# pinellolab/CRISPResso2

Hardware: NVIDIA H100
Metric: reads/sec aligned+classified (250 bp, single amplicon) (higher is better)
Workload: dtype int32

## Files before the change

### crispresso2_b200/_lib.py

```python
import ctypes as C
import os

import numpy as np

_HERE = os.path.dirname(os.path.abspath(__file__))
DEFAULT_LIB = os.path.join(_HERE, "libc2b200.so")

MAX_Q = 8
MAX_SEEDS = 8
MAX_READ_LEN = 512
MAX_REF_LEN = 1024

F_IGNORE_SUBSTITUTIONS = 1
F_IGNORE_INSERTIONS = 2
F_IGNORE_DELETIONS = 4
F_EXPAND_AMBIGUOUS = 8
F_ASSIGN_FIRST = 16
F_DISCARD_INDEL_READS = 32
F_NO_STRAND_SEARCH = 64
F_NO_PAIRING = 128
F_HDR_REF1 = 256
F_NO_RING = 512
F_LEGACY_INS = 1024
ANN_SAM_OPTIONAL = 1 << 16

ST_BAD_CHAR = 1
ST_UNDEFINED = 2
ST_EDIT_OVERFLOW = 4
E_ARG, E_LIMIT, E_STATE = -2, -3, -4
ST_TOO_LONG = 8

V_ALL_INS, V_ALL_INS_LEFT, V_ALL_DEL, V_ALL_SUB, V_INS, V_DEL, V_SUB, V_SUBBASE0 = range(8)
V_BASEDEV0 = V_SUBBASE0 + MAX_Q
V_INS_LEN = V_BASEDEV0 + MAX_Q + 1
V_DEL_LEN = V_INS_LEN + 1
V_R1_ALL_INS, V_R1_ALL_INS_LEFT, V_R1_ALL_DEL, V_R1_ALL_SUB = V_DEL_LEN + 1, V_DEL_LEN + 2, V_DEL_LEN + 3, V_DEL_LEN + 4
V_R1_BASEDEV0 = V_DEL_LEN + 5
V_INS_NONCODING = V_R1_BASEDEV0 + MAX_Q + 1
V_DEL_NONCODING, V_SUB_NONCODING = V_INS_NONCODING + 1, V_INS_NONCODING + 2
NVEC = V_INS_NONCODING + 3
H_INS_N, H_DEL_N, H_SUB_N, H_EFF_LEN, H_INFRAME, H_FRAMESHIFT, NHIST = range(7)
SCALARS = ["TOTAL", "MODIFIED", "UNMODIFIED", "DISCARDED", "INS", "DEL", "SUB", "ONLY_INS", "ONLY_DEL", "ONLY_SUB",
           "INS_DEL", "INS_SUB", "DEL_SUB", "INS_DEL_SUB", "AMBIGUOUS_W", "N_GLOBAL_SUBS", "N_SUBS_OUTSIDE_WINDOW",
           "N_MODS_IN_WINDOW", "N_MODS_OUTSIDE_WINDOW", "N_READS_IRREGULAR_ENDS", "N_ALIGNED_UNIQUE",
           "N_ALIGNED_COUNT", "REF1_W", "CLASS_MODIFIED", "CLASS_UNMODIFIED", "MOD_FRAMESHIFT", "MOD_NON_FRAMESHIFT",
           "NON_MOD_NON_FRAMESHIFT", "SPLICING_MODIFIED"]
NSCAL = len(SCALARS)
S = {n: k for k, n in enumerate(SCALARS)}


class Params(C.Structure):
    _fields_ = [("gap_open", C.c_int32), ("gap_extend", C.c_int32), ("seed_count", C.c_int32),
                ("seed_min", C.c_int32), ("flags", C.c_uint32), ("nq", C.c_int32),
                ("alphabet", C.c_char * MAX_Q), ("complement", C.c_uint8 * MAX_Q), ("edit_cap", C.c_int32)]


class Ref(C.Structure):
    _fields_ = [("seq", C.c_char_p), ("len", C.c_int32), ("gap_incentive", C.c_void_p),
                ("include_idx", C.c_void_p), ("n_include", C.c_int32), ("min_aln_score", C.c_double),
                ("score_rows", C.c_void_p), ("fw_seeds", C.POINTER(C.c_char_p)), ("rc_seeds", C.POINTER(C.c_char_p)),
                ("n_seeds", C.c_int32), ("tot_exon_len_mod", C.c_int32), ("coding_mask", C.c_void_p)]


ALN_DTYPE = np.dtype([("n_match", "<u2"), ("aln_len", "<u2"), ("score_milli", "<i4"), ("strand", "u1"),
                      ("status", "u1"), ("n_edits", "<u2"), ("insertion_n", "<u2"), ("deletion_n", "<u2"),
                      ("substitution_n", "<u2"), ("n_ins_all", "<u2"), ("n_ins_win", "<u2"), ("n_del_all", "<u2"),
                      ("n_del_win", "<u2"), ("n_del_pos_all", "<u2"), ("n_sub_all", "<u2"),
                      ("irregular_ends", "u1"), ("modified", "u1")])
REC_DTYPE = np.dtype([("winner_mask", "<u4"), ("best_score_milli", "<i4"), ("best_ref", "<i2"), ("n_winners", "u1"),
                      ("ambiguous", "u1"), ("status", "<u4")])
EDIT_DTYPE = np.dtype([("a", "<u2"), ("b", "<u2"), ("type", "u1"), ("in_window", "u1"), ("base", "u1"), ("pad", "u1")])
assert ALN_DTYPE.itemsize == 32 and REC_DTYPE.itemsize == 16 and EDIT_DTYPE.itemsize == 8

EXPORTS = ["c2b_create", "c2b_destroy", "c2b_last_error", "c2b_configure", "c2b_set_edit_cap", "c2b_string_width", "c2b_align_batch",
           "c2b_align_batch_compact", "c2b_ops_words", "c2b_expand_alignment", "c2b_expand_batch", "c2b_ops_device",
           "c2b_align_batch_device", "c2b_set_pair_order", "c2b_sync", "c2b_stream", "c2b_last_kernel_ms", "c2b_launch_count", "c2b_path_counts", "c2b_band_reruns", "c2b_ring_counts", "c2b_diag_counts", "c2b_route_counts",
           "c2b_counts_layout", "c2b_counts_hist_layout", "c2b_counts_reset", "c2b_counts_read", "c2b_counts_device", "c2b_global_align",
           "c2b_classify_aligned", "c2b_classify_aligned_flags", "c2b_host_alloc", "c2b_host_free",
           "c2b_fastq_dedup", "c2b_fastq_dedup_buffer", "c2b_fastq_gpu_available", "c2b_fastq_dedup_gpu", "c2b_fastq_dedup_gpu_buffer", "c2b_sam_dedup_gpu_buffer", "c2b_sam_dedup_buffer", "c2b_fastq_n_reads", "c2b_fastq_n_unique", "c2b_fastq_max_len",
           "c2b_fastq_seqs", "c2b_fastq_offsets", "c2b_fastq_counts", "c2b_fastq_first_index", "c2b_fastq_free",
           "c2b_fastq_last_error", "c2b_fastq_filter", "c2b_fastq_filter_pair", "c2b_rc_merge_weights", "c2b_screen_reads", "c2b_serial_stats",
           "c2b_consensus_from_pairs", "c2b_alleles_build", "c2b_alleles_free", "c2b_alleles_n", "c2b_alleles_order", "c2b_alleles_arena", "c2b_alleles_offsets",
           "c2b_alleles_lengths", "c2b_alleles_write_tsv", "c2b_alleles_around_cut", "c2b_alleles_cut_width", "c2b_alleles_cut_fetch",
           "c2b_annotate_build", "c2b_annotate_free", "c2b_annotate_n", "c2b_annotate_arena", "c2b_annotate_offsets",
           "c2b_annotate_cigar_arena", "c2b_annotate_cigar_offsets", "c2b_annotate_flags", "c2b_annotate_mapq", "c2b_annotate_first",
           "c2b_annotate_last_record", "c2b_annotate_record_arena", "c2b_annotate_record_offsets", "c2b_annotate_write_fastq",
           "c2b_annotate_write_sam", "c2b_annotate_write_sam_passthrough"]

_cache = {}


class LibraryMissing(ImportError):
    pass


def load(path=None):
    path = path or os.environ.get("C2B200_LIB") or DEFAULT_LIB
    if path in _cache:
        return _cache[path]
    if not os.path.exists(path):
        raise LibraryMissing("%s not found: build the CUDA extension first (python -c 'import __graft_entry__ as g; "
                             "g.build()'); crispresso2_b200 has no CPU fallback" % path)
    L = C.CDLL(path)
    vp, i32, i64 = C.c_void_p, C.c_int32, C.c_int64
    L.c2b_create.restype = C.c_int
    L.c2b_create.argtypes = [C.c_int, C.POINTER(vp)]
    L.c2b_destroy.restype = None
    L.c2b_destroy.argtypes = [vp]
    L.c2b_last_error.restype = C.c_char_p
    L.c2b_last_error.argtypes = [vp]
    L.c2b_configure.restype = C.c_int
    L.c2b_configure.argtypes = [vp, C.POINTER(Params), i32, C.POINTER(Ref)]
    L.c2b_set_edit_cap.restype = C.c_int
    L.c2b_set_edit_cap.argtypes = [vp, i32]
    L.c2b_string_width.restype = C.c_int
    L.c2b_string_width.argtypes = [vp, i32]
    L.c2b_align_batch.restype = C.c_int
    L.c2b_align_batch.argtypes = [vp, vp, vp, i64, vp, vp, vp, vp, vp, vp, vp]
    L.c2b_align_batch_compact.restype = C.c_int
    L.c2b_align_batch_compact.argtypes = [vp, vp, vp, i64, vp, vp, vp, vp, vp, vp, vp, vp]
    L.c2b_ops_words.restype = C.c_int
    L.c2b_ops_words.argtypes = [vp, i32]
    L.c2b_expand_alignment.restype = C.c_int
    L.c2b_expand_alignment.argtypes = [vp, vp, C.c_uint32, C.c_char_p, i32, C.c_char_p, i32, vp, vp]
    L.c2b_expand_batch.restype = C.c_int
    L.c2b_expand_batch.argtypes = [vp, vp, vp, i64, vp, vp, vp, i32, vp, i32]
    L.c2b_ops_device.restype = C.c_int
    L.c2b_ops_device.argtypes = [vp, C.POINTER(vp), C.POINTER(vp)]
    L.c2b_align_batch_device.restype = C.c_int
    L.c2b_align_batch_device.argtypes = [vp, vp, vp, i64, i32, vp, vp, vp, vp, vp, vp, vp]
    L.c2b_set_pair_order.restype = C.c_int
    L.c2b_set_pair_order.argtypes = [vp, vp]
    L.c2b_sync.restype = C.c_int
    L.c2b_sync.argtypes = [vp]
    L.c2b_stream.restype = vp
    L.c2b_stream.argtypes = [vp]
    L.c2b_last_kernel_ms.restype = C.c_double
    L.c2b_last_kernel_ms.argtypes = [vp]
    L.c2b_launch_count.restype = i64
    L.c2b_launch_count.argtypes = [vp]
    L.c2b_path_counts.restype = C.c_int
    L.c2b_path_counts.argtypes = [vp, C.POINTER(i64), C.POINTER(i64)]
    L.c2b_band_reruns.restype = i64
    L.c2b_band_reruns.argtypes = [vp]
    L.c2b_ring_counts.restype = C.c_int
    L.c2b_ring_counts.argtypes = [vp, C.POINTER(i64), C.POINTER(i64)]
    L.c2b_diag_counts.restype = C.c_int
    L.c2b_diag_counts.argtypes = [vp, C.POINTER(i64), C.POINTER(i64), C.POINTER(i64)]
    L.c2b_route_counts.restype = C.c_int
    L.c2b_route_counts.argtypes = [vp, C.POINTER(i64), C.POINTER(i64)]
    L.c2b_counts_layout.restype = C.c_int
    L.c2b_counts_layout.argtypes = [vp, C.POINTER(i32), C.POINTER(i32), C.POINTER(i32), C.POINTER(i32)]
    L.c2b_counts_hist_layout.restype = C.c_int
    L.c2b_counts_hist_layout.argtypes = [vp, C.POINTER(i32), C.POINTER(i32), C.POINTER(i32)]
    L.c2b_counts_reset.restype = C.c_int
    L.c2b_counts_reset.argtypes = [vp]
    L.c2b_counts_read.restype = C.c_int
    L.c2b_counts_read.argtypes = [vp, vp, C.c_size_t]
    L.c2b_counts_device.restype = C.c_int
    L.c2b_counts_device.argtypes = [vp, C.POINTER(vp), C.POINTER(C.c_size_t)]
    L.c2b_global_align.restype = C.c_int
    L.c2b_global_align.argtypes = [vp, C.c_char_p, i32, C.c_char_p, i32, C.c_char_p, i32, vp, vp, i32, i32,
                                   C.c_char_p, C.c_char_p, C.POINTER(i32), C.POINTER(i32)]
    L.c2b_classify_aligned.restype = C.c_int
    L.c2b_classify_aligned.argtypes = [vp, C.c_char_p, C.c_char_p, i32, C.c_char_p, i32, vp, i32, vp, vp]
    L.c2b_classify_aligned_flags.restype = C.c_int
    L.c2b_classify_aligned_flags.argtypes = [vp, C.c_char_p, C.c_char_p, i32, C.c_char_p, i32, vp, i32, C.c_uint32, vp, vp]
    L.c2b_host_alloc.restype = vp
    L.c2b_host_alloc.argtypes = [C.c_size_t]
    L.c2b_host_free.restype = None
    L.c2b_host_free.argtypes = [vp]
    L.c2b_fastq_dedup.restype = C.c_int
    L.c2b_fastq_dedup.argtypes = [C.c_char_p, i32, C.POINTER(vp)]
    L.c2b_fastq_dedup_buffer.restype = C.c_int
    L.c2b_fastq_dedup_buffer.argtypes = [vp, C.c_size_t, i32, C.POINTER(vp)]
    for name, rt in (("c2b_fastq_n_reads", i64), ("c2b_fastq_n_unique", i64), ("c2b_fastq_max_len", i32),
                     ("c2b_fastq_seqs", vp), ("c2b_fastq_offsets", vp), ("c2b_fastq_counts", vp),
                     ("c2b_fastq_first_index", vp)):
        getattr(L, name).restype = rt
        getattr(L, name).argtypes = [vp]
    L.c2b_fastq_free.restype = None
    L.c2b_fastq_free.argtypes = [vp]
    L.c2b_consensus_from_pairs.restype = C.c_int
    L.c2b_consensus_from_pairs.argtypes = [C.c_char_p, i32, C.c_char_p, i32, C.c_double, C.c_char_p, i32,
                                           C.c_char_p, i32, C.c_char_p, i32, C.c_double, C.c_char_p, i32,
                                           C.c_char_p, C.c_char_p, C.c_char_p, i32,
                                           C.POINTER(i32), C.POINTER(i32), C.POINTER(i32), C.POINTER(i32)]
    L.c2b_fastq_gpu_available.restype = C.c_int
    L.c2b_fastq_gpu_available.argtypes = []
    L.c2b_fastq_dedup_gpu.restype = C.c_int
    L.c2b_fastq_dedup_gpu.argtypes = [C.c_char_p, i32, C.POINTER(vp)]
    L.c2b_fastq_dedup_gpu_buffer.restype = C.c_int
    L.c2b_fastq_dedup_gpu_buffer.argtypes = [vp, C.c_size_t, i32, C.POINTER(vp)]
    L.c2b_sam_dedup_gpu_buffer.restype = C.c_int
    L.c2b_sam_dedup_gpu_buffer.argtypes = [vp, C.c_size_t, i32, C.POINTER(vp)]
    L.c2b_sam_dedup_buffer.restype = C.c_int
    L.c2b_sam_dedup_buffer.argtypes = [vp, C.c_size_t, i32, C.POINTER(vp)]
    L.c2b_fastq_filter.restype = C.c_int
    L.c2b_fastq_filter.argtypes = [C.c_char_p, C.c_char_p, i32, i32, i32, i32, C.POINTER(i64), C.POINTER(i64)]
    L.c2b_fastq_filter_pair.restype = C.c_int
    L.c2b_fastq_filter_pair.argtypes = [C.c_char_p, C.c_char_p, C.c_char_p, C.c_char_p, i32, i32, i32, i32, C.POINTER(i64), C.POINTER(i64)]
    L.c2b_rc_merge_weights.restype = C.c_int
    L.c2b_rc_merge_weights.argtypes = [vp, vp, i64, vp, vp, vp, i32]
    L.c2b_screen_reads.restype = i64
    L.c2b_screen_reads.argtypes = [vp, vp, i64, i32, vp, i32]
    L.c2b_fastq_last_error.restype = C.c_char_p
    L.c2b_fastq_last_error.argtypes = []
    L.c2b_serial_stats.restype = C.c_int
    L.c2b_serial_stats.argtypes = [vp, vp, vp, i64, i32, vp, vp, i32]
    L.c2b_alleles_build.restype = C.c_int
    L.c2b_alleles_build.argtypes = [vp, vp, vp, vp, i32, i64, vp, vp, vp, vp, i32, C.POINTER(C.c_char_p), vp, vp, i32, C.POINTER(vp)]
    L.c2b_alleles_free.restype = None
    L.c2b_alleles_free.argtypes = [vp]
    L.c2b_alleles_n.restype = i64
    L.c2b_alleles_n.argtypes = [vp]
    for name in ("c2b_alleles_order", "c2b_alleles_arena", "c2b_alleles_offsets", "c2b_alleles_lengths"):
        getattr(L, name).restype = vp
        getattr(L, name).argtypes = [vp]
    L.c2b_alleles_write_tsv.restype = C.c_int
    L.c2b_alleles_write_tsv.argtypes = [vp, C.c_char_p, i64, vp, vp, C.POINTER(C.c_char_p), vp, C.POINTER(C.c_char_p), vp, vp, vp, vp,
                                        C.POINTER(C.c_char_p), i32]
    L.c2b_alleles_around_cut.restype = i64
    L.c2b_alleles_around_cut.argtypes = [vp, i64, vp, i32, i32, i32, vp, vp, vp, vp, vp]
    L.c2b_alleles_cut_width.restype = i32
    L.c2b_alleles_cut_width.argtypes = [vp]
    L.c2b_alleles_cut_fetch.restype = C.c_int
    L.c2b_alleles_cut_fetch.argtypes = [vp, vp, vp, vp, vp, vp, vp, vp, vp, vp]
    cpp = C.POINTER(C.c_char_p)
    L.c2b_annotate_build.restype = C.c_int
    L.c2b_annotate_build.argtypes = [vp, vp, vp, i64, vp, i32, i32, i32, vp, vp, vp, vp, vp, vp, vp, vp, i32, cpp, vp, i32, cpp, cpp, vp,
                                     vp, C.c_uint32, i64, C.POINTER(vp)]
    L.c2b_annotate_free.restype = None
    L.c2b_annotate_free.argtypes = [vp]
    L.c2b_annotate_n.restype = i64
    L.c2b_annotate_n.argtypes = [vp]
    for name in ("c2b_annotate_arena", "c2b_annotate_offsets", "c2b_annotate_cigar_arena", "c2b_annotate_cigar_offsets",
                 "c2b_annotate_flags", "c2b_annotate_mapq", "c2b_annotate_first", "c2b_annotate_last_record",
                 "c2b_annotate_record_arena", "c2b_annotate_record_offsets"):
        getattr(L, name).restype = vp
        getattr(L, name).argtypes = [vp]
    L.c2b_annotate_write_fastq.restype = C.c_int
    L.c2b_annotate_write_fastq.argtypes = [vp, vp, vp, i64, C.c_char_p, C.c_char_p, i32]
    L.c2b_annotate_write_sam.restype = C.c_int
    L.c2b_annotate_write_sam.argtypes = [vp, vp, vp, i64, C.c_char_p, C.c_char_p, C.c_char_p, i32, cpp, cpp, vp, i32]
    L.c2b_annotate_write_sam_passthrough.restype = C.c_int
    L.c2b_annotate_write_sam_passthrough.argtypes = [vp, vp, vp, i64, vp, C.c_size_t, C.c_char_p, i32]
    _cache[path] = L
    return L
```

### crispresso2_b200/csrc/c2b_core.cuh

```cuda
#pragma once
#include <stdint.h>
#include "c2b200.h"

#ifndef C2B_EMU
#include <cuda_runtime.h>
#define C2B_DEV __device__ __forceinline__
#define C2B_DEVNOINL __device__ __noinline__
namespace wp {
C2B_DEV int lane() { return threadIdx.x & 31; }
C2B_DEV int shfl_up(int v, int d) { return __shfl_up_sync(0xffffffffu, v, d); }
C2B_DEV int shfl(int v, int src) { return __shfl_sync(0xffffffffu, v, src); }
C2B_DEV uint32_t shflu(uint32_t v, int src) { return __shfl_sync(0xffffffffu, v, src); }
C2B_DEV uint32_t shflu_up(uint32_t v, int d) { return __shfl_up_sync(0xffffffffu, v, d); }
C2B_DEV int shfl_xor(int v, int m) { return __shfl_xor_sync(0xffffffffu, v, m); }
C2B_DEV uint32_t ballot(bool p) { return __ballot_sync(0xffffffffu, p); }
C2B_DEV void sync() { __syncwarp(); }
#ifdef C2B_X_INLINE_BARRIER
C2B_DEV
#else
__device__ __noinline__
#endif
void grp_sync(int g)
{
    const int w = (int)(threadIdx.x >> 5), sh = 31 - __clz(g);
    const int set = w >> sh;
    asm volatile("barrier.sync %0, %1;" ::"r"(1 + set), "r"(32 << sh) : "memory");
}
C2B_DEV int max3(int a, int b, int c) { return __vimax3_s32(a, b, c); }
C2B_DEV int addmax(int a, int b, int c) { return __viaddmax_s32(a, b, c); }
C2B_DEV uint32_t max3_2(uint32_t a, uint32_t b, uint32_t c) { return __vimax3_s16x2(a, b, c); }
C2B_DEV uint32_t addmax_2(uint32_t a, uint32_t b, uint32_t c) { return __viaddmax_s16x2(a, b, c); }
C2B_DEV uint4 ldg4u(const uint4 *p) { return __ldg(p); }
C2B_DEV void prefetch_l2(const void *p) { asm volatile("prefetch.global.L2 [%0];" ::"l"(p)); }
C2B_DEV int grid_warps() { return (int)(gridDim.x * (blockDim.x >> 5)); }
C2B_DEV uint32_t smem_addr(const void *p) { return (uint32_t)__cvta_generic_to_shared(p); }
C2B_DEV uint32_t lds_u8(uint32_t a) { uint32_t v; asm volatile("ld.shared.u8 %0, [%1];" : "=r"(v) : "r"(a)); return v; }
C2B_DEV uint4 lds_v4(uint32_t a) { uint4 v; asm volatile("ld.shared.v4.u32 {%0,%1,%2,%3}, [%4];" : "=r"(v.x), "=r"(v.y), "=r"(v.z), "=r"(v.w) : "r"(a)); return v; }
C2B_DEV uint2 ldcg2(const uint2 *p) { return __ldcg(p); }
C2B_DEV uint32_t funnel_r(uint32_t lo, uint32_t hi, int sh) { return __funnelshift_r(lo, hi, sh); }
C2B_DEV int popc(uint32_t x) { return __popc(x); }
C2B_DEV int popcll(uint64_t x) { return __popcll(x); }
C2B_DEV int clz(uint32_t x) { return __clz(x); }
C2B_DEV int ffs(uint32_t x) { return __ffs(x); }
C2B_DEV uint32_t ldcg(const uint32_t *p) { return __ldcg(p); }
C2B_DEV int ldcgi(const int *p) { return __ldcg(p); }
C2B_DEV uint64_t ldcg64(const uint64_t *p) { return __ldcg((const unsigned long long *)p); }
C2B_DEV int4 ldg4(const int4 *p) { return __ldg(p); }
C2B_DEV void addg(unsigned long long *p, long long v)
{ asm volatile("red.global.add.u64 [%0], %1;" ::"l"(__cvta_generic_to_global(p)), "l"((unsigned long long)v) : "memory"); }
C2B_DEV void maxg(unsigned long long *p, unsigned long long v)
{ asm volatile("red.global.max.u64 [%0], %1;" ::"l"(__cvta_generic_to_global(p)), "l"(v) : "memory"); }
C2B_DEV uint32_t adds(uint32_t *p, uint32_t v)
{ uint32_t o; asm volatile("atom.shared.add.u32 %0, [%1], %2;" : "=r"(o) : "r"((uint32_t)__cvta_generic_to_shared(p)), "r"(v) : "memory"); return o; }
C2B_DEV unsigned long long fetch_work(unsigned long long *p)
{ unsigned long long o; asm volatile("atom.global.add.u64 %0, [%1], %2;" : "=l"(o) : "l"(__cvta_generic_to_global(p)), "l"(1ull) : "memory"); return o; }
C2B_DEV unsigned long long fetch_add(unsigned long long *p, unsigned long long v)
{ unsigned long long o; asm volatile("atom.global.add.u64 %0, [%1], %2;" : "=l"(o) : "l"(__cvta_generic_to_global(p)), "l"(v) : "memory"); return o; }
}

#else
#include "warp_emu.h"
namespace wp {
C2B_DEV int grid_warps() { return 1; }
}
#endif

namespace c2b {

constexpr int MAXJ = C2B_MAX_READ_LEN;
constexpr int MAXI = C2B_MAX_REF_LEN;
constexpr int OP_M = 0, OP_J = 1, OP_I = 2, OP_NONE = 3;

struct RefDev {
    int32_t I, nrb, kstar, lstar, Ipad;
    int32_t gi0_4;
    int32_t nseeds, seed_len;
    double min_aln;
    const int32_t *prof;
    const int32_t *cIe;
    const int32_t *g4;
    const uint8_t *asc;
    const uint8_t *rcode;
    const uint8_t *incl;
    const uint16_t *cum;
    const uint16_t *cumx, *cums;
    int32_t coding, tem, hist_zero;
    unsigned long long *hist;
    uint64_t fw_seed[C2B_MAX_SEEDS], rc_seed[C2B_MAX_SEEDS];
    unsigned long long *vec;
    unsigned long long *scal;
    int32_t pk_maxJ;
    uint32_t pk_XB, pk_YB, pk_M00;
    const uint32_t *prof2;
    const uint32_t *cIe2;
    const uint32_t *g42;
    int32_t rg_ok, rg_smax, rg_gmax, rg_gsum;
    int32_t dg_ok, dg_S, dg_thr4;
    int32_t dg_c4[2 * 4 + 1];
    int32_t rt_ok, rt_thr;
    int32_t rt_mx;
    int32_t rt_c[32];
    const uint4 *rt_pl;
};
constexpr int32_t RT_OFF = -(1 << 30);
constexpr int RN_DLO = 17, RN_DHI = 11;

struct WorkBlock {
    unsigned long long pair_items, single_items, band_reruns, ring_kept, ring_sent, align_settled;
    unsigned long long diag_proved, diag_listed, tier2, routed, kept;
    struct Launch {
        unsigned long long align_next, tier2_next, general_next;
        unsigned long long widest;
        unsigned long long left_n, tier2_n, narrow_n, diag_n;
    } launch;
};
constexpr size_t WORK_BYTES = 32 * 8;
static_assert(sizeof(WorkBlock) <= WORK_BYTES, "work block");

struct KParams {
    const uint8_t *reads; const int64_t *offsets; int64_t n_reads;
    const int32_t *count, *qweight, *ref_id;
    const int32_t *pair_order;
    c2b_read_rec *recs; c2b_aln_rec *alns; uint8_t *strings; c2b_edit *edits;
    int32_t W, edit_cap;
    const RefDev *refs; int32_t n_refs;
    int32_t out_refs, ops_refs;
    int32_t go, ge, seed_count, seed_min; uint32_t flags; int32_t nq;
    uint8_t alpha[C2B_MAX_Q]; uint8_t comp[C2B_MAX_Q];
    uint32_t *tb; int64_t tb_words_per_warp; int32_t TS;
    uint32_t *tbb; int64_t tbb_words_per_warp;
    uint32_t *tbq;
    int32_t *bnd; int64_t bnd_words_per_warp;
    uint64_t *opsbuf;
    uint64_t *rgops;
    WorkBlock *wb;
    unsigned long long *work_counter;
    uint64_t *gops; uint32_t *gmeta; int32_t NW;
    int32_t *left;
    int32_t *left2;
    int32_t *left0;
    int32_t *left1;
    int32_t route;
    const unsigned long long *n_dev;
    int32_t vstride, hstride;
    const uint32_t *stage_src;
    int32_t stage_bytes;
    const uint8_t *lut;
    int32_t phase_sync;
    const uint64_t *forced_ops;
    const int32_t *forced_n;
};

C2B_DEV int64_t oslot(const KParams &P, int64_t rd, int r) { return rd * P.out_refs + (P.ref_id ? 0 : r); }
C2B_DEV int64_t nreads(const KParams &P) { return P.n_dev ? (int64_t)*P.n_dev : P.n_reads; }

C2B_DEV const RefDev &refdev(const KParams &P, int r) { return P.refs[r]; }

struct WarpSmem {
    uint8_t fw[2][MAXJ];
    uint8_t rc[2][MAXJ];
    uint8_t combo[MAXJ];
    uint8_t rowinfo[MAXI];
    uint32_t rowins[MAXI + 4];
};
constexpr int PK_ROWINFO_STRIDE = 512, PK_ROWINS_STRIDE = 514, PK_MAX_ALN = 512, PK_MAX_ALN2 = 1024;
constexpr int RG_NS = 72, RG_B = 32, RG_MAXD = 8, RG_COMBO = 320;
constexpr int RG_MAX_REFS = 4, RG_OPS_STRIDE = 36;
constexpr int RG_DLO = RG_B + 1, RG_DHI = RG_NS - RG_B - 9;
struct QuadSmem {
    union {
        uint8_t combo[4][RG_COMBO];
        struct { uint64_t ops[4][32]; int32_t n[4][2], err[4][2]; } wk;
    };
};
constexpr int PK_BAND_SLOTS = 64, PK_BAND_B = 28, PK_BAND_MAXD = 8;
struct SlabMode { int slope, off, ns, ring, gb; };

struct Walked { uint64_t ops; int n; int err; uint64_t ops2; };

template <int KSTAR>
C2B_DEV void dp_block(const KParams &P, const RefDev &R, const uint8_t *codes, const int J, const int rb, const int NEG4,
                      uint32_t *__restrict__ tb, const int32_t *bnd_in, int32_t *bnd_out, int &cM, int &cX, int &cY)
{
    const int lane = wp::lane();
    const int nrb = R.nrb, lstar = R.lstar, Ipad = R.Ipad, gi0_4 = R.gi0_4;
    const bool lastblk = (rb == nrb - 1);
    const int nl = lastblk ? lstar + 1 : 32;
    const int rowbase = rb * 256;
    const int r0 = rowbase + 8 * lane;
    const bool islast = lastblk && lane == lstar;
    const int ge4 = 4 * P.ge, d4 = 4 * (P.go - P.ge);

    int M[8], X[8], Y[8], cIe[8], g4[8];
    {
        const int4 *pc = reinterpret_cast<const int4 *>(R.cIe + r0);
        const int4 *pg = reinterpret_cast<const int4 *>(R.g4 + r0);
        int4 a = wp::ldg4(pc), b = wp::ldg4(pc + 1), c = wp::ldg4(pg), d = wp::ldg4(pg + 1);
        cIe[0] = a.x; cIe[1] = a.y; cIe[2] = a.z; cIe[3] = a.w; cIe[4] = b.x; cIe[5] = b.y; cIe[6] = b.z; cIe[7] = b.w;
        g4[0] = c.x; g4[1] = c.y; g4[2] = c.z; g4[3] = c.w; g4[4] = d.x; g4[5] = d.y; g4[6] = d.z; g4[7] = d.w;
    }
#pragma unroll
    for (int k = 0; k < 8; k++) {
        M[k] = NEG4; X[k] = NEG4 | 2; Y[k] = (ge4 * (r0 + k + 1) + gi0_4) | 1;
    }
    int pM, pX, pY;
    if (rb == 0) { pM = 0; pX = NEG4 | 2; pY = NEG4 | 1; }
    else { pM = NEG4; pX = NEG4 | 2; pY = (ge4 * rowbase + gi0_4) | 1; }

    const int nsteps = J + nl - 1;
    const int32_t *__restrict__ prof0 = R.prof + r0;
    uint32_t *__restrict__ tbw = tb + ((int64_t)rb * P.TS) * 32 + lane;
    const bool lane_on = lane < nl;
    int topX = gi0_4 | 2;

    for (int t = 1; t <= nsteps; t++) {
        int uM = wp::shfl_up(M[7], 1), uX = wp::shfl_up(X[7], 1), uY = wp::shfl_up(Y[7], 1);
        const int j = t - lane;
        if (lane == 0) {
            if (rb == 0) { topX += ge4; uM = NEG4; uX = topX; uY = NEG4 | 1; }
            else if (j <= J) { uM = wp::ldcgi(bnd_in + 3 * j); uX = wp::ldcgi(bnd_in + 3 * j + 1); uY = wp::ldcgi(bnd_in + 3 * j + 2); }
        }
        if (lane_on && j >= 1 && j <= J) {
            const int q = codes[j - 1];
            const int4 *pp = reinterpret_cast<const int4 *>(prof0 + q * Ipad);
            const int4 sa = wp::ldg4(pp), sb = wp::ldg4(pp + 1);
            const int s[8] = {sa.x, sa.y, sa.z, sa.w, sb.x, sb.y, sb.z, sb.w};
            const int dcol = (j == J) ? 0 : d4;
            const int dsp = islast ? 0 : dcol;
            int dM = pM, dX = pX, dY = pY;
            int upM = uM, upY = uY;
            uint32_t wT = 0, wIJ = 0;
#pragma unroll
            for (int k = 0; k < 8; k++) {
                const int dik = (k == KSTAR) ? dsp : dcol;
                const int z = wp::max3(dM, dY, dX);
                const int tag = z & 3;
                const int nm = (z - tag) + s[k];
                const int x = wp::addmax(M[k], dik, X[k]) + cIe[k];
                const int y = wp::addmax(upM, dik + g4[k], upY) + ge4;
                wT = wp::funnel_r(wT, (uint32_t)z, 2);
                wIJ = wp::funnel_r(wIJ, (uint32_t)(x | y), 2);
                dM = M[k]; dX = X[k]; dY = Y[k];
                M[k] = nm; X[k] = x | 2; Y[k] = y | 1;
                upM = nm; upY = Y[k];
            }
            tbw[(int64_t)t * 32] = (wT & 0xffff0000u) | (wIJ >> 16);
            if (!lastblk && lane == 31) { bnd_out[3 * j] = M[7]; bnd_out[3 * j + 1] = X[7]; bnd_out[3 * j + 2] = Y[7]; }
        }
        pM = uM; pX = uX; pY = uY;
    }
    if (lastblk) {
        const int k = (KSTAR < 8) ? KSTAR : 0;
        cM = wp::shfl(M[k], lstar); cX = wp::shfl(X[k], lstar); cY = wp::shfl(Y[k], lstar);
    }
}

C2B_DEV void dp_dispatch(const KParams &P, const RefDev &R, const uint8_t *codes, int J, int rb, int NEG4,
                         uint32_t *tb, const int32_t *bi, int32_t *bo, int &cM, int &cX, int &cY)
{
    const int ks = (rb == R.nrb - 1) ? R.kstar : 8;
    switch (ks) {
    case 0: dp_block<0>(P, R, codes, J, rb, NEG4, tb, bi, bo, cM, cX, cY); break;
// ... 1343 lines not shown
```

### crispresso2_b200/csrc/c2b_engine.cu

```cuda
#include <algorithm>
#include <atomic>
#include <mutex>
#ifndef C2B_EMU
#include <sched.h>
#include <sys/syscall.h>
#include <unistd.h>
#include <cctype>
#endif
#include <chrono>
#include <cstdio>
#include <cstdlib>
#include <cstring>
#include <string>
#include <thread>
#include <vector>

#include "c2b_core.cuh"
#include "c2b_split.cuh"
#include "c2b_annotate.cuh"
#include "c2b_fastq_int.h"

using namespace c2b;

#ifndef C2B_EMU
// ... 415 lines not shown
    e->n_refs = n_refs;
    e->refs.assign(n_refs, RefHost());
    e->refdev.assign(n_refs, RefDev());
    int maxI = 0, max_nrb = 1;
    size_t bytes = 0;
    auto al = [](size_t x) { return (x + 255) & ~(size_t)255; };
    std::vector<size_t> base(n_refs);
    for (int r = 0; r < n_refs; r++) {
        const c2b_ref &rf = refs[r];
        if (!rf.seq || rf.len < 1 || !rf.gap_incentive || !rf.score_rows) return fail(e, C2B_E_ARG, "c2b_configure: incomplete reference");
        if (rf.len > C2B_MAX_REF_LEN) return fail(e, C2B_E_LIMIT, "c2b_configure: reference longer than C2B_MAX_REF_LEN");
        if (rf.n_seeds > 0 && (!rf.fw_seeds || !rf.rc_seeds)) return fail(e, C2B_E_ARG, "c2b_configure: seeds missing");
        maxI = std::max(maxI, rf.len);
        const int nrb = (rf.len + 255) / 256, Ipad = nrb * 256;
        max_nrb = std::max(max_nrb, nrb);
        base[r] = bytes;
        bytes += al((size_t)p->nq * Ipad * 4) + 2 * al((size_t)Ipad * 4) + 2 * al(Ipad) + al(Ipad + 1) + 3 * al((size_t)(Ipad + 2) * 2);
        bytes += al((size_t)p->nq * p->nq * Ipad * 4) + 2 * al((size_t)Ipad * 4);
        bytes += al((size_t)(Ipad / 32 + 2) * 16);
    }
    const size_t refs_off = bytes;
    bytes += al(sizeof(RefDev) * n_refs);
    std::vector<unsigned char> blob(bytes, 0);
    if (e->d_tables) { rt_free(e->d_tables); e->d_tables = nullptr; }
    RTCHK(rt_malloc(&e->d_tables, bytes));
    e->vstride = (maxI + 31) & ~31;
    {
        int max_tem = 0;
        for (int r = 0; r < n_refs; r++) max_tem = std::max(max_tem, std::abs((int)refs[r].tot_exon_len_mod));
        if (max_tem > 4 * C2B_MAX_REF_LEN) return fail(e, C2B_E_LIMIT, "c2b_configure: tot_exon_len_mod out of range");
        e->hist_zero = maxI + max_tem;
        const int need = std::max(e->hist_zero + C2B_MAX_READ_LEN + max_tem, std::min(maxI + C2B_MAX_READ_LEN, C2B_MAX_ALN_LEN)) + 1;
        e->hstride = (need + 31) & ~31;
    }
    const size_t per_ref = C2B_NVEC * (size_t)e->vstride + C2B_NHIST * (size_t)e->hstride + C2B_NSCAL;
    e->counts_n = (size_t)n_refs * per_ref;
    if (e->d_counts) { rt_free(e->d_counts); e->d_counts = nullptr; }
    RTCHK(rt_malloc((void **)&e->d_counts, e->counts_n * 8));
    RTCHK(rt_zero(e->d_counts, e->counts_n * 8, e->stream));

    for (int r = 0; r < n_refs; r++) {
        const c2b_ref &rf = refs[r];
        const int I = rf.len, nrb = (I + 255) / 256, Ipad = nrb * 256;
        RefDev &d = e->refdev[r];
        e->refs[r].seq.assign(rf.seq, (size_t)rf.len);
        d.I = I; d.nrb = nrb; d.Ipad = Ipad; d.kstar = (I - 1) & 7; d.lstar = ((I - 1) >> 3) & 31;
        d.min_aln = rf.min_aln_score;
        unsigned char *hb = blob.data() + base[r];
        unsigned char *db = (unsigned char *)e->d_tables + base[r];
        size_t o = 0;
        int32_t *prof = (int32_t *)(hb + o); d.prof = (const int32_t *)(db + o); o += al((size_t)p->nq * Ipad * 4);
        int32_t *cIe = (int32_t *)(hb + o); d.cIe = (const int32_t *)(db + o); o += al((size_t)Ipad * 4);
        int32_t *g4 = (int32_t *)(hb + o); d.g4 = (const int32_t *)(db + o); o += al((size_t)Ipad * 4);
        uint8_t *asc = hb + o; d.asc = db + o; o += al(Ipad);
        uint8_t *rcode = hb + o; d.rcode = db + o; o += al(Ipad);
        uint8_t *incl = hb + o; d.incl = db + o; o += al(Ipad + 1);
        uint16_t *cum = (uint16_t *)(hb + o); d.cum = (const uint16_t *)(db + o); o += al((size_t)(Ipad + 2) * 2);
        uint16_t *cumx = (uint16_t *)(hb + o); d.cumx = (const uint16_t *)(db + o); o += al((size_t)(Ipad + 2) * 2);
        uint16_t *cums = (uint16_t *)(hb + o); d.cums = (const uint16_t *)(db + o); o += al((size_t)(Ipad + 2) * 2);
        uint32_t *prof2 = (uint32_t *)(hb + o); d.prof2 = (const uint32_t *)(db + o); o += al((size_t)p->nq * p->nq * Ipad * 4);
        uint32_t *cIe2 = (uint32_t *)(hb + o); d.cIe2 = (const uint32_t *)(db + o); o += al((size_t)Ipad * 4);
        uint32_t *g42 = (uint32_t *)(hb + o); d.g42 = (const uint32_t *)(db + o); o += al((size_t)Ipad * 4);
        uint4 *rt_pl = (uint4 *)(hb + o); d.rt_pl = (const uint4 *)(db + o); o += al((size_t)(Ipad / 32 + 2) * 16);
        const int64_t lim = (1ll << 27);
        for (int q = 0; q < p->nq; q++)
            for (int i = 0; i < I; i++) {
                const int64_t v = rf.score_rows[(size_t)q * I + i];
                if (v > lim || v < -lim) return fail(e, C2B_E_LIMIT, "c2b_configure: substitution score out of range");
                prof[(size_t)q * Ipad + i] = (int32_t)(4 * v);
            }
        for (int i = 0; i <= I; i++) if (rf.gap_incentive[i] > lim || rf.gap_incentive[i] < -lim) return fail(e, C2B_E_LIMIT, "c2b_configure: gap incentive out of range");
        {
            RefHost &h = e->refs[r];
            h.sabs = h.gabs = h.gsum_abs = 0; h.gi0_abs = std::abs(rf.gap_incentive[0]);
            for (size_t k = 0; k < (size_t)p->nq * I; k++) h.sabs = std::max<int64_t>(h.sabs, std::abs(rf.score_rows[k]));
            for (int i = 0; i <= I; i++) { h.gabs = std::max<int64_t>(h.gabs, std::abs(rf.gap_incentive[i])); h.gsum_abs += std::abs(rf.gap_incentive[i]); }
        }
        for (int row = 0; row < I; row++) {
            cIe[row] = (int32_t)(4 * (p->gap_extend + rf.gap_incentive[row + 1]));
            g4[row] = (int32_t)(4 * rf.gap_incentive[row]);
            asc[row] = (uint8_t)rf.seq[row];
            int code = 255;
            for (int q = 0; q < p->nq; q++) if (rf.seq[row] == p->alphabet[q]) code = q;
            rcode[row] = (uint8_t)code;
        }
        d.gi0_4 = (int32_t)(4 * rf.gap_incentive[0]);
        {
            const int64_t go = p->gap_open, ge = p->gap_extend, beta = -ge, OFFu = 512;
            int64_t gmin = rf.gap_incentive[0], gmax = rf.gap_incentive[0], smin = rf.score_rows[0], smax = rf.score_rows[0];
            for (int i = 0; i <= I; i++) { gmin = std::min(gmin, rf.gap_incentive[i]); gmax = std::max(gmax, rf.gap_incentive[i]); }
            for (size_t k = 0; k < (size_t)p->nq * I; k++) { smin = std::min(smin, rf.score_rows[k]); smax = std::max(smax, rf.score_rows[k]); }
            bool ok = go <= ge && ge <= 0 && gmin >= 0 && gmax <= 64 && smin + 2 * beta >= 0 && smax + 2 * beta <= 1000 &&
                      (go - ge) > -1900 && 4 * (OFFu + (go - ge)) > 256 + 4 * gmax + 3 + 64 && !(p->flags & C2B_F_NO_PAIRING);
            d.pk_maxJ = 0;
            if (ok) {
                for (int J = 1; J <= C2B_MAX_READ_LEN && I + J <= PK_MAX_ALN2; J++) {
                    const int64_t bound = 4 * ((smax + 2 * beta) * std::min(I, J) + gmax * (I + J + 2) + OFFu) + 3;
                    if (bound > 32000) break;
                    d.pk_maxJ = J;
                }
            }
            const uint32_t rep = 0x00010001u;
            d.pk_XB = (uint32_t)((4 * (rf.gap_incentive[0] + OFFu)) | 2) * rep;
            d.pk_YB = (uint32_t)((4 * (rf.gap_incentive[0] + OFFu)) | 1) * rep;
            d.pk_M00 = (uint32_t)(4 * OFFu) * rep;
            {
                int64_t gsum = 0;
                for (int i = 0; i <= I; i++) gsum += rf.gap_incentive[i];
                d.rg_smax = (int32_t)smax; d.rg_gmax = (int32_t)gmax; d.rg_gsum = (int32_t)std::min<int64_t>(gsum, 1 << 24);
                d.rg_ok = d.pk_maxJ > 0 && nrb == 1 && smax >= 0 && 2 * ge + gmax <= smax && gsum < (1 << 24) && !(p->flags & C2B_F_NO_RING);
            }
            if (d.pk_maxJ > 0) {
                for (int qa = 0; qa < p->nq; qa++)
                    for (int qb = 0; qb < p->nq; qb++)
                        for (int i = 0; i < I; i++) {
                            const uint32_t a = (uint32_t)(4 * (rf.score_rows[(size_t)qa * I + i] + 2 * beta));
                            const uint32_t b = (uint32_t)(4 * (rf.score_rows[(size_t)qb * I + i] + 2 * beta));
                            const int rbk = i >> 8, ln = (i >> 3) & 31, hf = (i >> 2) & 1, wd = i & 3;
                            prof2[((size_t)qa * p->nq + qb) * Ipad + rbk * 256 + hf * 128 + ln * 4 + wd] = a | (b << 16);
                        }
                for (int row = 0; row < I; row++) {
                    cIe2[row] = (uint32_t)(4 * rf.gap_incentive[row + 1]) * rep;
                    g42[row] = (uint32_t)(4 * rf.gap_incentive[row]) * rep;
                }
            }
        }
        for (int k = 0; k < rf.n_include; k++) {
            const int64_t v = rf.include_idx[k];
            if (v >= 0 && v < I) incl[v] = 1;
        }
        cum[0] = 0;
        for (int q = 0; q <= Ipad; q++) cum[q + 1] = (uint16_t)(cum[q] + (q < I && incl[q] ? 1 : 0));
        d.coding = rf.coding_mask != nullptr; d.tem = rf.tot_exon_len_mod; d.hist_zero = e->hist_zero;
        {
            const int64_t go = p->gap_open, ge = p->gap_extend, gi0 = rf.gap_incentive[0], gI = rf.gap_incentive[I];
            int64_t gmin = gi0, gp = 0, smax = rf.score_rows[0];
            for (int i = 0; i <= I; i++) { gmin = std::min(gmin, rf.gap_incentive[i]); gp = std::max(gp, rf.gap_incentive[i]); }
            for (size_t k = 0; k < (size_t)p->nq * I; k++) smax = std::max(smax, rf.score_rows[k]);
            int64_t thr = smax * (I - 1) + go + ge + 2 * gp;
            thr = std::max(thr, go * I * I + std::max<int64_t>(smax, 0) * I + 2 * (int64_t)I * gp);
            auto edge_bound = [&](int64_t t) { return smax * (I - t) + t * (2 * ge + gp) + gp; };
            int S = 0;
            while (S < 4 && S + 1 < I && edge_bound(S + 1) > thr) S++;
            if (S + 1 < I) thr = std::max(thr, edge_bound(S + 1));
            thr = std::max<int64_t>(thr, -(1ll << 28));
            d.dg_ok = d.rg_ok && !d.coding && go <= ge && ge <= 0 && gmin >= 0 && 2 * (ge + gp) <= smax && I >= 2 && thr < (1ll << 28) &&
                      !(p->flags & C2B_F_NO_RING);
            d.dg_S = S; d.dg_thr4 = (int32_t)(4 * thr);
            for (int s = -4; s <= 4; s++) {
                const int64_t t = s < 0 ? -s : s;
                d.dg_c4[s + 4] = (int32_t)(4 * (s == 0 ? 0 : 2 * ge * t + gi0 + (s > 0 ? rf.gap_incentive[I - std::min<int64_t>(t, I)] : t * gI)));
            }
            if (!d.dg_ok) { d.dg_S = 0; d.dg_thr4 = 0; }
        }
        {
            const int nq4 = std::min(p->nq, 4);
            for (int i = 0; i < I; i++) {
                const int q = rcode[i];
                if (q >= nq4) continue;
                uint4 &w = rt_pl[i >> 5];
                const uint32_t bit = 1u << (i & 31);
                if (q & 1) w.x |= bit;
                if (q & 2) w.y |= bit;
                w.z |= bit;
            }
            int64_t m = INT64_MAX, x = INT64_MAX;
            for (int q = 0; q < p->nq; q++)
                for (int i = 0; i < I; i++) {
                    const int64_t v = rf.score_rows[(size_t)q * I + i];
                    if (q == rcode[i] && q < nq4) m = std::min(m, v); else x = std::min(x, v);
                }
            const int64_t ge = p->gap_extend, go = p->gap_open, smax = d.rg_smax, gmax = d.rg_gmax, gsum = d.rg_gsum;
            int64_t thr = -(1 << 28);
            if (RN_DHI + 1 <= I) thr = std::max(thr, smax * (I - RN_DHI - 1) + (RN_DHI + 1) * (ge + gmax) + (RN_DHI + 1) * ge + gsum);
            if (RN_DLO + 1 <= I) thr = std::max(thr, smax * (I - RN_DLO - 1) + (RN_DLO + 1) * (ge + gmax) + (RN_DLO + 1) * ge + gsum);
            const int64_t gI = rf.gap_incentive[I];
            const int64_t big = std::max<int64_t>({std::abs(m == INT64_MAX ? 0 : m), std::abs(x == INT64_MAX ? 0 : x), std::abs(go), std::abs(ge), e->refs[r].gabs});
            d.rt_ok = d.dg_ok && I <= 256 && m != INT64_MAX && x != INT64_MAX && m > x && big * (4 * I + 64) < (1ll << 28);
            d.rt_thr = d.rt_ok ? (int32_t)thr : 0;
            d.rt_mx = d.rt_ok ? (int32_t)(m - x) : 0;
            for (int k = 0; k < 32; k++) {
                const int s = k - 16, t = s < 0 ? -s : s;
                const bool on = d.rt_ok && s != 0 && t < I && (s < 0 ? t <= RN_DLO : t <= RN_DHI);
                d.rt_c[k] = RT_OFF;
                if (on) d.rt_c[k] = (int32_t)(go + (t - 1) * ge + (s < 0 ? t * (ge + gI) : t * ge + rf.gap_incentive[I - t]) + x * (I - t));
            }
        }
        if (rf.coding_mask)
            for (int q = 0; q < I; q++) incl[q] |= (uint8_t)((rf.coding_mask[q] & 3) << 1);
        cumx[0] = cums[0] = 0;
        for (int q = 0; q <= Ipad; q++) {
            cumx[q + 1] = (uint16_t)(cumx[q] + (q < I && (incl[q] & 2) ? 1 : 0));
            cums[q + 1] = (uint16_t)(cums[q] + (q < I && (incl[q] & 4) ? 1 : 0));
        }
        const int ns = std::min({(int)rf.n_seeds, (int)p->seed_count, (int)C2B_MAX_SEEDS});
        if (rf.n_seeds > 0 && std::min((int)rf.n_seeds, (int)p->seed_count) > C2B_MAX_SEEDS)
            return fail(e, C2B_E_LIMIT, "c2b_configure: more seeds than C2B_MAX_SEEDS");
        d.nseeds = ns; d.seed_len = 0;
        for (int s = 0; s < C2B_MAX_SEEDS; s++) { d.fw_seed[s] = ~0ull; d.rc_seed[s] = ~0ull; }
        for (int s = 0; s < ns; s++) {
            const std::string f = rf.fw_seeds[s], c = rf.rc_seeds[s];
            if (f.size() != c.size() || f.empty() || f.size() > C2B_MAX_SEED_LEN) return fail(e, C2B_E_LIMIT, "c2b_configure: seed length unsupported");
            if (s && (int)f.size() != d.seed_len) return fail(e, C2B_E_LIMIT, "c2b_configure: seeds of unequal length");
            d.seed_len = (int)f.size();
            d.fw_seed[s] = pack_seed(*p, f); d.rc_seed[s] = pack_seed(*p, c);
        }
        d.vec = e->d_counts + (size_t)r * per_ref;
        d.hist = d.vec + C2B_NVEC * (size_t)e->vstride;
        d.scal = d.hist + C2B_NHIST * (size_t)e->hstride;
    }
    memcpy(blob.data() + refs_off, e->refdev.data(), sizeof(RefDev) * n_refs);
    e->d_refs = (RefDev *)((unsigned char *)e->d_tables + refs_off);
    RTCHK(rt_h2d(e->d_tables, blob.data(), bytes, e->stream));
    RTCHK(rt_sync(e->stream));
    {
        unsigned char lut[256];
        memset(lut, 255, sizeof lut);
        for (int q = 0; q < p->nq; q++) lut[(unsigned char)p->alphabet[q]] = (unsigned char)q;
        int rc2;
        if ((rc2 = ensure(e, e->lut, 256))) return rc2;
        RTCHK(rt_h2d(e->lut.p, lut, 256, e->stream));
        RTCHK(rt_sync(e->stream));
    }
    e->max_I = maxI; e->max_nrb = max_nrb;
    {
        int n_ok = 0;
        for (int r = 0; r < n_refs; r++) n_ok += (e->refdev[r].pk_maxJ > 0 && !e->refdev[r].coding) ? 1 : 0;
        e->split_ok = !(p->flags & (C2B_F_NO_PAIRING | C2B_F_NO_RING)) && n_ok > 0;
        e->split_all = n_ok == n_refs;
        e->diag_any = 0;
        for (int r = 0; r < n_refs; r++) e->diag_any |= e->refdev[r].dg_ok ? 1 : 0;
    }
    e->scratch_TS = 0;
    e->configured = true;
    return C2B_OK;
}

int c2b_set_edit_cap(c2b_engine *e, int32_t edit_cap)
{
    if (!e || !e->configured || edit_cap < 0) return fail(e, C2B_E_ARG, "c2b_set_edit_cap: bad argument");
    e->prm.edit_cap = edit_cap;
    return C2B_OK;
}

int c2b_string_width(const c2b_engine *e, int32_t max_read_len)
{
    if (!e || !e->configured) return C2B_E_STATE;
    return (e->max_I + max_read_len + 31) & ~31;
}

static int ensure_scratch(c2b_engine *e, int maxJ)
{
    const int TS = ((maxJ + 32 + 31) & ~31);
    if (TS <= e->scratch_TS) return C2B_OK;
    int rc;
    auto al = [](size_t x) { return (x + 255) & ~(size_t)255; };
    if ((rc = ensure(e, e->tb, al((size_t)e->n_warps * e->max_nrb * TS * 64 * 4)))) return rc;
    if ((rc = ensure(e, e->tbb, al((size_t)e->n_warps * PK_BAND_SLOTS * 64 * 4)))) return rc;
    if ((rc = ensure(e, e->tbq, al((size_t)e->n_warps * TS * 64 * 4 + 64)))) return rc;
    if ((rc = ensure(e, e->bnd, al((size_t)e->n_warps * 2 * 3 * TS * 4)))) return rc;
    if ((rc = ensure(e, e->ops, al((size_t)e->n_warps * std::min(e->n_refs, (int)C2B_MAX_REFS) * 32 * 8)))) return rc;
    if ((rc = ensure(e, e->rgo, al((size_t)e->n_warps * RG_MAX_REFS * 4 * RG_OPS_STRIDE * 8)))) return rc;
    const bool fresh_work = !e->work.p;
    if ((rc = ensure(e, e->work, WORK_BYTES))) return rc;
    if (fresh_work) RTCHK(rt_zero(e->work.p, WORK_BYTES, e->stream));
    e->scratch_TS = TS;
    return C2B_OK;
}

static int score_range_ok(c2b_engine *e, int64_t maxJ, const char *who)
{
    const int64_t go = std::abs((int64_t)e->prm.gap_open), gap = std::max(go, std::abs((int64_t)e->prm.gap_extend));
    for (int r = 0; r < e->n_refs; r++) {
        const RefHost &h = e->refs[r];
        const int64_t I = (int64_t)h.seq.size(), J = std::max<int64_t>(maxJ, 1);
        const int64_t bound = go * I * J + std::min(I, J) * h.sabs + (I + J) * gap + J * h.gabs + h.gsum_abs + h.gi0_abs;
        if (4 * bound + 3 > (int64_t)INT32_MAX)
            return fail(e, C2B_E_LIMIT, std::string(who) + ": scores, gap penalties and incentives can exceed the int32 range of the DP");
    }
    return C2B_OK;
}

struct Batch {
    const uint8_t *reads; const int64_t *offsets; int64_t n_reads; int32_t max_read_len;
    const int32_t *count, *qweight, *ref_id;
    c2b_read_rec *recs; c2b_aln_rec *alns; uint8_t *strings; c2b_edit *edits;
    uint64_t *gops; uint32_t *gmeta; int32_t *left, *left2, *left0, *left1;
};

struct Switches { bool no_diag, no_route, route_all, no_narrow, no_split; };
static Switches read_switches()
{
    return {getenv("C2B_NO_DIAG") != nullptr, getenv("C2B_NO_ROUTE") != nullptr, getenv("C2B_ROUTE_ALL") != nullptr,
            getenv("C2B_NO_NARROW") != nullptr, getenv("C2B_NO_SPLIT") != nullptr};
}

enum StepKind { STEP_DIAG, STEP_ALIGN, STEP_CLASSIFY, STEP_GENERAL };
struct Step { StepKind kind; KParams P; int grid, block; size_t smem; };
struct Plan { Step step[5]; int n = 0; bool one = false; };

static Plan plan_batch(const c2b_engine *e, const Batch &b, const Switches &sw)
{
    Plan plan;
    WorkBlock *wb = (WorkBlock *)e->work.p;
    KParams P;
    memset(&P, 0, sizeof P);
// ... 92 lines not shown
        wp::g_grp_syncs = 0;
        if (one) emu::run_warp([&]() { process_group<true>(P, S, Q, nullptr, w, 0); });
        else emu::run_warp([&]() { process_group<false>(P, S, Q, nullptr, w, 0); });
        if (P.phase_sync && wp::g_grp_syncs != group_phases(P)) {
            fprintf(stderr, "warp_emu: work group %lld executed %ld phase barriers, expected %d\n", (long long)w, wp::g_grp_syncs, group_phases(P));
            abort();
        }
    }
}

static int run_plan(c2b_engine *, const Plan &plan, rt_stream)
{
    static WarpSmem S; static QuadSmem Q; static ASmem AS; static BSmem BS; static DSmem DS;
    for (int k = 0; k < plan.n; k++) {
        const KParams &P = plan.step[k].P;
        switch (plan.step[k].kind) {
        case STEP_DIAG: emu::run_warp([&]() { diag_loop(P, DS, 0, 1); }); break;
        case STEP_ALIGN: emu::run_warp([&]() { align_loop(P, AS, nullptr, 0); }); break;
        case STEP_CLASSIFY:
            if (plan.one) emu::run_warp([&]() { classify_loop<true>(P, BS, 0, 1); });
            else emu::run_warp([&]() { classify_loop<false>(P, BS, 0, 1); });
            break;
        case STEP_GENERAL:
            if (P.n_dev && plan.one) emu::run_warp([&]() { general_list_loop<true>(P, S, nullptr, 0); });
            else if (P.n_dev) emu::run_warp([&]() { general_list_loop<false>(P, S, nullptr, 0); });
            else run_phase_sets(P, plan.one, S, Q);
            break;
        }
    }
    return C2B_OK;
}
#endif

static int launch_on(c2b_engine *e, rt_stream cs, Batch b)
{
    if (!e || !e->configured) return fail(e, C2B_E_STATE, "c2b_align_batch: engine not configured");
    if (b.n_reads < 0 || !b.recs || !b.alns || (b.n_reads && (!b.reads || !b.offsets))) return fail(e, C2B_E_ARG, "c2b_align_batch: bad argument");
    if (b.n_reads >= (1ll << 31)) return fail(e, C2B_E_LIMIT, "c2b_align_batch: more than 2^31 reads in one batch");
    if (b.max_read_len < 1) b.max_read_len = 1;
    if (b.max_read_len > C2B_MAX_READ_LEN) return fail(e, C2B_E_LIMIT, "c2b_align_batch: read longer than C2B_MAX_READ_LEN");
    if ((int64_t)std::abs((long long)e->prm.gap_open) * b.max_read_len * e->max_I >= (1ll << 28))
        return fail(e, C2B_E_LIMIT, "c2b_align_batch: gap_open * lengths exceeds the int32 score range");
    if (int rc0 = score_range_ok(e, b.max_read_len, "c2b_align_batch")) return rc0;
    if (!b.ref_id && e->n_refs > C2B_MAX_REFS)
        return fail(e, C2B_E_LIMIT, "c2b_align_batch: more than C2B_MAX_REFS references need a per-read ref_id");
    int rc = ensure_scratch(e, b.max_read_len);
    if (rc) return rc;
    if (b.n_reads == 0) return C2B_OK;
    const Plan plan = plan_batch(e, b, read_switches());
    RTCHK(rt_zero(&((WorkBlock *)e->work.p)->launch, sizeof(WorkBlock::Launch), cs));
    if (b.gmeta) RTCHK(rt_zero(b.gmeta, (size_t)b.n_reads * (b.ref_id ? 1 : e->n_refs) * 4, cs));
    if ((rc = run_plan(e, plan, cs))) return rc;
    e->launches += plan.n;
    return C2B_OK;
}

static int ensure_ops(c2b_engine *e, DevBuf &gops, DevBuf &gmeta, DevBuf &left, DevBuf &left2, DevBuf &left0, DevBuf &left1, int64_t n_reads,
                      int nr, int W)
{
    int rc;
    if ((rc = ensure(e, gops, (size_t)n_reads * nr * (W / 32) * 8))) return rc;
    if ((rc = ensure(e, gmeta, (size_t)n_reads * nr * 4))) return rc;
    if ((rc = ensure(e, left, (size_t)(n_reads + 8) * 4))) return rc;
    if ((rc = ensure(e, left2, (size_t)(n_reads + 16) * 4))) return rc;
    if ((rc = ensure(e, left0, (size_t)(n_reads + 16) * 4))) return rc;
    if ((rc = ensure(e, left1, (size_t)(n_reads + 16) * 4))) return rc;
    return C2B_OK;
}

int c2b_align_batch_device(c2b_engine *e, const uint8_t *d_reads, const int64_t *d_offsets, int64_t n_reads,
                           int32_t max_read_len, const int32_t *d_count, const int32_t *d_qweight,
                           const int32_t *d_ref_id, c2b_read_rec *d_recs, c2b_aln_rec *d_alns,
                           uint8_t *d_strings, c2b_edit *d_edits)
{
    if (!e || !e->configured) return fail(e, C2B_E_STATE, "c2b_align_batch_device: engine not configured");
#ifndef C2B_EMU
    cudaSetDevice(e->device);
#endif
    if (max_read_len < 1) max_read_len = 1;
    const int W = (e->max_I + max_read_len + 31) & ~31, nr = d_ref_id ? 1 : e->n_refs;
    int rc = ensure_ops(e, e->gops, e->gmeta, e->left, e->left2, e->left0, e->left1, n_reads, nr, W);
    if (rc) return rc;
    return launch_on(e, e->stream, Batch{d_reads, d_offsets, n_reads, max_read_len, d_count, d_qweight, d_ref_id, d_recs,
                     d_alns, d_strings, d_edits, (uint64_t *)e->gops.p, (uint32_t *)e->gmeta.p, (int32_t *)e->left.p, (int32_t *)e->left2.p,
                     (int32_t *)e->left0.p, (int32_t *)e->left1.p});
}

int c2b_ops_device(c2b_engine *e, void **d_ops, void **d_meta)
{
    if (!e) return C2B_E_ARG;
    if (d_ops) *d_ops = e->gops.p;
    if (d_meta) *d_meta = e->gmeta.p;
    return C2B_OK;
}

int64_t c2b_band_reruns(c2b_engine *e) { return e ? e->band_reruns : 0; }

int c2b_set_pair_order(c2b_engine *e, const int32_t *d_order)
{
    if (!e) return C2B_E_ARG;
    e->pair_order = d_order;
    return C2B_OK;
}

int c2b_sync(c2b_engine *e)
{
    if (!e) return C2B_E_ARG;
    RTCHK(rt_sync(e->stream));
    return C2B_OK;
}

void *c2b_stream(c2b_engine *e) { return e ? (void *)(uintptr_t)e->stream : nullptr; }

double c2b_last_kernel_ms(c2b_engine *e)
{
#ifndef C2B_EMU
    if (!e || !e->launches) return 0.0;
    float ms = 0.f;
    if (cudaEventSynchronize(e->ev1) != cudaSuccess) return 0.0;
    if (cudaEventElapsedTime(&ms, e->ev0, e->ev1) != cudaSuccess) return 0.0;
    return (double)ms;
#else
    (void)e; return 0.0;
#endif
}

int64_t c2b_launch_count(const c2b_engine *e) { return e ? e->launches : 0; }

int c2b_path_counts(c2b_engine *e, int64_t *pair_items, int64_t *single_items)
{
    if (!e || !e->work.p) return fail(e, C2B_E_STATE, "c2b_path_counts: nothing launched yet");
    WorkBlock v;
    RTCHK(rt_d2h(&v, e->work.p, sizeof v, e->stream));
    RTCHK(rt_sync(e->stream));
    e->band_reruns = (int64_t)v.band_reruns; e->ring_pairs = (int64_t)(v.ring_kept + 1) / 2; e->ring_fallbacks = (int64_t)(v.ring_sent + 1) / 2;
    if (getenv("C2B_VERBOSE"))
        fprintf(stderr, "[c2b] counters: general kernel %lld pair items + %lld single items; ALIGN: %lld read x reference combinations kept "
                        "by the ring, %lld sent to the full matrix, %lld reads settled\n", (long long)v.pair_items, (long long)v.single_items,
                (long long)v.ring_kept, (long long)v.ring_sent, (long long)v.align_settled);
    if (pair_items) *pair_items = (int64_t)(v.pair_items + (v.align_settled + 1) / 2);
    if (single_items) *single_items = (int64_t)v.single_items;
    return C2B_OK;
}

int c2b_diag_counts(c2b_engine *e, int64_t *proved, int64_t *tier1, int64_t *tier2)
{
    if (!e || !e->work.p) return fail(e, C2B_E_STATE, "c2b_diag_counts: nothing launched yet");
    WorkBlock v;
    RTCHK(rt_d2h(&v, e->work.p, sizeof v, e->stream));
    RTCHK(rt_sync(e->stream));
    if (proved) *proved = (int64_t)v.diag_proved;
    if (tier1) *tier1 = (int64_t)v.diag_listed;
    if (tier2) *tier2 = (int64_t)v.tier2;
    return C2B_OK;
}

int c2b_route_counts(c2b_engine *e, int64_t *routed, int64_t *kept)
{
    if (!e || !e->work.p) return fail(e, C2B_E_STATE, "c2b_route_counts: nothing launched yet");
    WorkBlock v;
    RTCHK(rt_d2h(&v, e->work.p, sizeof v, e->stream));
    RTCHK(rt_sync(e->stream));
    if (routed) *routed = (int64_t)v.routed;
    if (kept) *kept = (int64_t)v.kept;
    return C2B_OK;
}

int c2b_ring_counts(c2b_engine *e, int64_t *ring_pairs, int64_t *ring_fallbacks)
{
    if (!e) return C2B_E_ARG;
    if (ring_pairs) *ring_pairs = e->ring_pairs;
    if (ring_fallbacks) *ring_fallbacks = e->ring_fallbacks;
    return C2B_OK;
}

static bool is_pageable(const void *p)
{
#ifndef C2B_EMU
    if (!p) return false;
    cudaPointerAttributes a;
    if (cudaPointerGetAttributes(&a, p) != cudaSuccess) { cudaGetLastError(); return true; }
    return a.type == cudaMemoryTypeUnregistered;
#else
    (void)p; return false;
#endif
}

static void par_copy2d(void *dst, size_t dpitch, const void *src, size_t spitch, size_t width, size_t rows)
{
    if (!rows || !width) return;
    const size_t bytes = width * rows;
    int T = bytes > (8u << 20) ? 4 : bytes > (1u << 20) ? 2 : 1;
    auto work = [&](int t) {
        const size_t lo = rows * t / T, hi = rows * (t + 1) / T;
        if (dpitch == width && spitch == width) memcpy((char *)dst + lo * width, (const char *)src + lo * width, (hi - lo) * width);
        else for (size_t r = lo; r < hi; r++) memcpy((char *)dst + r * dpitch, (const char *)src + r * spitch, width);
    };
    std::vector<std::thread> th;
    for (int t = 1; t < T; t++) th.emplace_back(work, t);
    work(0);
    for (auto &x : th) x.join();
}
static void par_copy(void *dst, const void *src, size_t bytes) { par_copy2d(dst, bytes, src, bytes, bytes, 1 == 1 ? (bytes ? 1 : 0) : 0); }

static int ensure_pinned(c2b_engine *e, uint8_t *&p, size_t &cap, size_t n)
{
    if (n <= cap) return C2B_OK;
    if (p) rt_host_free(p);
    const size_t want = n + n / 8 + 4096;
    p = (uint8_t *)rt_host_alloc(want); cap = p ? want : 0;
    return p ? C2B_OK : fail(e, C2B_E_CUDA, "c2b_align_batch: pinned allocation failed");
}

static int align_batch_host(c2b_engine *e, const uint8_t *reads, const int64_t *offsets, int64_t n_reads,
                            const int32_t *count, const int32_t *qweight, const int32_t *ref_id,
                            c2b_read_rec *recs, c2b_aln_rec *alns, uint8_t *strings, uint64_t *ops, uint32_t *meta, c2b_edit *edits)
{
    if (!e || !e->configured) return fail(e, C2B_E_STATE, "c2b_align_batch: engine not configured");
    if (n_reads < 0 || !recs || !alns || (n_reads && (!reads || !offsets))) return fail(e, C2B_E_ARG, "c2b_align_batch: bad argument");
    if ((ops == nullptr) != (meta == nullptr)) return fail(e, C2B_E_ARG, "c2b_align_batch: ops and meta go together");
#ifndef C2B_EMU
    cudaSetDevice(e->device);
#endif
    if (n_reads == 0) return C2B_OK;
    int64_t maxJ = 1, minJ = 0;
    for (int64_t r = 0; r < n_reads; r++) {
        const int64_t L = offsets[r + 1] - offsets[r];
        maxJ = L > maxJ ? L : maxJ;
        minJ = L < minJ ? L : minJ;
    }
    if (minJ < 0) return fail(e, C2B_E_ARG, "c2b_align_batch: offsets not monotone");
    if (maxJ > C2B_MAX_READ_LEN) return fail(e, C2B_E_LIMIT, "c2b_align_batch: read longer than C2B_MAX_READ_LEN");
    if (int rc0 = score_range_ok(e, maxJ, "c2b_align_batch")) return rc0;
    if (!e->pipe_ready) {
        RTCHK(rt_stream_create(&e->s_in));
        RTCHK(rt_stream_create(&e->s_out));
        for (auto &st : e->stage) { RTCHK(rt_event_create(&st.in_done)); RTCHK(rt_event_create(&st.k_done)); RTCHK(rt_event_create(&st.out_done)); }
        e->pipe_ready = true;
    }
    const int W = (e->max_I + (int)maxJ + 31) & ~31, NW = W / 32;
    const int cap = edits ? e->prm.edit_cap : 0;
    const int nr = ref_id ? 1 : e->n_refs;
    const int64_t per_read = (int64_t)nr * (2 * (int64_t)W * (strings ? 1 : 0) + NW * 8 + (int64_t)cap * 8 + 36) + 16 + maxJ + 28;
    int64_t chunk = std::max<int64_t>(4096, std::min<int64_t>((int64_t)(1536ll << 20) / per_read, 1 << 18));
    if (n_reads < 4 * chunk) chunk = std::max<int64_t>(4096, (n_reads + 3) / 4);
    if (const char *v = getenv("C2B_CHUNK")) chunk = std::max<int64_t>(2, atoll(v));
    for (auto &st : e->stage) st.used = false;
    int rc = C2B_OK;
    const bool bounce = getenv("C2B_FORCE_BOUNCE") ? atoi(getenv("C2B_FORCE_BOUNCE")) != 0 : (is_pageable(reads) || is_pageable(recs));
    auto al256 = [](size_t x) { return (x + 255) & ~(size_t)255; };
    struct OutLay { size_t recs, alns, ed, meta, str, ops, total; };
    auto out_layout = [&](int64_t n) {
        OutLay L; size_t o = 0;
        L.recs = o; o = al256(o + (size_t)n * sizeof(c2b_read_rec));
        L.alns = o; o = al256(o + (size_t)n * nr * sizeof(c2b_aln_rec));
        L.ed = o; o = al256(o + (size_t)n * nr * cap * sizeof(c2b_edit));
        L.meta = o; o = al256(o + (meta ? (size_t)n * nr * 4 : 0));
        L.str = o; o = al256(o + (strings ? (size_t)n * nr * 2 * W : 0));
        L.ops = o; o = al256(o + (ops ? (size_t)n * nr * NW * 8 : 0));
        L.total = o;
        return L;
    };
    struct Pending { bool any = false; int64_t c0 = 0, n = 0; int set = 0; } pend;
    auto flush = [&](const Pending &q) -> int {
        c2b_engine::Stage &st = e->stage[q.set];
        const OutLay L = out_layout(q.n);
        int rc2;
        if (bounce && (rc2 = ensure_pinned(e, st.h_out, st.h_out_cap, L.total))) return rc2;
        uint8_t *ho = st.h_out;
        RTCHK(rt_wait(e->s_out, st.k_done));
        RTCHK(rt_d2h(bounce ? (void *)(ho + L.recs) : (void *)(recs + q.c0), st.recs.p, (size_t)q.n * sizeof(c2b_read_rec), e->s_out));
        RTCHK(rt_d2h(bounce ? (void *)(ho + L.alns) : (void *)(alns + q.c0 * nr), st.alns.p, (size_t)q.n * nr * sizeof(c2b_aln_rec), e->s_out));
        if (cap) RTCHK(rt_d2h(bounce ? (void *)(ho + L.ed) : (void *)(edits + q.c0 * nr * cap), st.ed.p, (size_t)q.n * nr * cap * sizeof(c2b_edit), e->s_out));
        if (meta) RTCHK(rt_d2h(bounce ? (void *)(ho + L.meta) : (void *)(meta + q.c0 * nr), st.gmeta.p, (size_t)q.n * nr * 4, e->s_out));
        size_t Wt = 0;
        if (strings || ops) {
            RTCHK(rt_event_sync(st.k_done));
            long long wmax = 0;
            RTCHK(rt_d2h(&wmax, (const char *)st.maxlen.p, 8, e->s_out));
            RTCHK(rt_sync(e->s_out));
            Wt = ((size_t)wmax + 31) & ~(size_t)31;
            if (Wt > (size_t)W) Wt = W;
            if (strings) RTCHK(rt_d2h_2d((bounce ? ho + L.str : strings + q.c0 * nr * 2 * W) + (W - Wt), (const uint8_t *)st.str.p + (W - Wt), W, Wt, (size_t)q.n * nr * 2, e->s_out));
            if (ops) RTCHK(rt_d2h_2d(bounce ? (void *)(ho + L.ops) : (void *)(ops + q.c0 * nr * NW), st.gops.p, (size_t)NW * 8, Wt / 32 * 8, (size_t)q.n * nr, e->s_out));
        }
        RTCHK(rt_record(st.out_done, e->s_out));
        st.drain = bounce; st.d_c0 = q.c0; st.d_n = q.n; st.d_Wt = Wt;
        return C2B_OK;
    };
    auto drain = [&](c2b_engine::Stage &st) -> int {
        if (!st.drain) return C2B_OK;
        RTCHK(rt_event_sync(st.out_done));
        const int64_t c0 = st.d_c0, n = st.d_n;
        const OutLay L = out_layout(n);
        const uint8_t *ho = st.h_out;
        par_copy(recs + c0, ho + L.recs, (size_t)n * sizeof(c2b_read_rec));
        par_copy(alns + c0 * nr, ho + L.alns, (size_t)n * nr * sizeof(c2b_aln_rec));
        if (cap) par_copy(edits + c0 * nr * cap, ho + L.ed, (size_t)n * nr * cap * sizeof(c2b_edit));
        if (meta) par_copy(meta + c0 * nr, ho + L.meta, (size_t)n * nr * 4);
        if (strings) par_copy2d(strings + c0 * nr * 2 * W + (W - st.d_Wt), W, ho + L.str + (W - st.d_Wt), W, st.d_Wt, (size_t)n * nr * 2);
        if (ops) par_copy2d(ops + c0 * nr * NW, (size_t)NW * 8, ho + L.ops, (size_t)NW * 8, st.d_Wt / 32 * 8, (size_t)n * nr);
        st.drain = false;
        return C2B_OK;
    };
    std::vector<int64_t> cuts;
    {
// ... 480 lines not shown
```

### crispresso2_b200/csrc/c2b_split.cuh

```cuda
#pragma once
#include "c2b_core.cuh"

namespace c2b {

constexpr uint32_t GM_NONE = 0, GM_ALIGNED = 1;

C2B_DEV uint32_t gmeta_pack(int n, int strand, uint32_t state) { return (uint32_t)n | ((uint32_t)strand << 16) | (state << 24); }

struct ASmem {
    uint8_t fw[2][RG_COMBO], rc[2][RG_COMBO];
    uint8_t combo[8][RG_COMBO];
    uint32_t fin[96];
    uint8_t lut[256];
};

C2B_DEV void asmem_init(const KParams &P, ASmem &S)
{
    const int lane = wp::lane();
    for (int k = lane; k < 256; k += 32) S.lut[k] = P.lut[k];
    wp::sync();
}

C2B_DEV int64_t read_at(const KParams &P, int64_t idx) { return P.pair_order ? (int64_t)P.pair_order[idx] : idx; }

C2B_DEV void leftover_pair(const KParams &P, int64_t rdA, int64_t rdB)
{
    if (wp::lane() == 0) {
        const unsigned long long pos = wp::fetch_add(&P.wb->launch.left_n, 2ull);
        P.left[pos] = (int32_t)rdA; P.left[pos + 1] = (int32_t)rdB;
    }
}

C2B_DEV void leftover_one(const KParams &P, int64_t rd)
{
    if (wp::lane() == 0) { const unsigned long long pos = wp::fetch_add(&P.wb->launch.left_n, 1ull); P.left[pos] = (int32_t)rd; }
}

C2B_DEV bool load_codes_a(const KParams &P, const uint8_t *lut, int64_t off, int J, uint8_t *fw, uint8_t *rc)
{
    const int lane = wp::lane();
    bool bad = false;
    for (int base = 0; base < J; base += 128) {
        uint8_t ch[4];
#pragma unroll
        for (int e = 0; e < 4; e++) { const int p = base + lane + 32 * e; ch[e] = p < J ? P.reads[off + p] : (uint8_t)P.alpha[0]; }
#pragma unroll
        for (int e = 0; e < 4; e++) {
            const int p = base + lane + 32 * e;
            int code = lut[ch[e]];
            if (code == 255) { bad = true; code = 0; }
            if (p < J) { fw[p] = (uint8_t)code; rc[J - 1 - p] = P.comp[code]; }
        }
    }
    return wp::ballot(bad) != 0;
}

template <int RL = 8, int NP = 4>
C2B_DEV void walk_ring4(const KParams &P, const RefDev &R, const int *Jq, const uint2 *__restrict__ tb2, const int *s0, uint32_t mask,
                        Walked *out, const int q0 = 0)
{
    constexpr int NS = 9 * RL, B = 4 * RL;
    const int lane = wp::lane();
    const int hl = lane & 15, hb = lane & 16;
    const int TS = P.TS;
    int i[NP], j[NP], s[NP], n[NP], err[NP];
    uint32_t acc[NP], lo[NP], hi[NP];
#pragma unroll
    for (int q = 0; q < NP; q++) {
        const bool on = (mask >> q) & 1u;
        i[q] = on ? R.I : 0; j[q] = on ? Jq[q] : 0; s[q] = s0[q]; n[q] = 0; err[q] = 0; acc[q] = 0; lo[q] = hi[q] = ~0u;
    }
#define C2B_PUSH4(q, op_, cnt_) do { int cnt = (cnt_); const uint32_t pat = (uint32_t)(op_) * 0x55555555u;                          \
        while (cnt > 0) { const int room = 16 - (n[q] & 15); const int c = cnt < room ? cnt : room;                                  \
            acc[q] = (uint32_t)((((uint64_t)pat << 32) | acc[q]) >> (2 * c)); n[q] += c; cnt -= c;                                   \
            if ((n[q] & 15) == 0) { const int ix = (n[q] >> 4) - 1; if (hl == (ix >> 1)) { if (ix & 1) hi[q] = acc[q]; else lo[q] = acc[q]; } } } } while (0)
    for (;;) {
        uint2 w2[NP]; bool valid[NP], inband[NP]; int sh[NP];
        bool anyact = false;
#pragma unroll
        for (int q = 0; q < NP; q++) {
            const bool active = i[q] > 0 && j[q] > 0;
            anyact |= active;
            const int di = (s[q] != OP_I), dj = (s[q] != OP_J);
            const int ci = i[q] - hl * di, cj = j[q] - hl * dj;
            valid[q] = active && ci >= 1 && cj >= 1;
            inband[q] = valid[q];
            w2[q] = make_uint2(0u, 0u); sh[q] = 0;
            if (valid[q]) {
                const int r = ci - 1, l = (r >> 3) & 31;
                const int slot = cj + l - 9 * l + B;
                inband[q] = (unsigned)slot < (unsigned)NS;
                sh[q] = 2 * (7 - (r & 7));
                if (inband[q]) w2[q] = wp::ldcg2(tb2 + (int64_t)(RL * (q0 + q) + (l & (RL - 1))) * TS + cj + l);
            }
        }
        if (!wp::ballot(anyact)) break;
#pragma unroll
        for (int q = 0; q < NP; q++) {
            const bool active = i[q] > 0 && j[q] > 0;
            const uint32_t w = hb ? ((w2[q].x & 0xffff0000u) | (w2[q].y >> 16)) : ((w2[q].x << 16) | (w2[q].y & 0xffffu));
            const uint32_t v = (valid[q] && inband[q]) ? (w >> sh[q]) : 0u;
            const int tag = (int)((v >> 16) & 3u);
            const bool cont = valid[q] && (s[q] == OP_M ? tag == OP_M : (v & (uint32_t)s[q]) != 0u);
            const uint32_t bc = (wp::ballot(cont) >> hb) & 0xffffu, bv = (wp::ballot(valid[q]) >> hb) & 0xffffu;
            const uint32_t bo = (wp::ballot(valid[q] && !inband[q]) >> hb) & 0xffffu;
            int nvalid = wp::popc(bv);
            if (bo) { const int fo = wp::ffs(bo) - 1; if (fo < nvalid) nvalid = fo; }
            const bool miss = active && nvalid == 0;
            int f = wp::ffs(~bc) - 1;
            if (f < 0 || f > nvalid) f = nvalid;
            const bool brk = f < nvalid;
            const int run = brk ? f + 1 : nvalid;
            const int tagf = wp::shfl(tag, hb + (f < 16 ? f : 15));
            if (miss) { err[q] |= 4; i[q] = 0; j[q] = 0; }
            else if (active) {
                const int di = (s[q] != OP_I), dj = (s[q] != OP_J);
                const int news = brk ? (s[q] == OP_M ? tagf : OP_M) : s[q];
                C2B_PUSH4(q, s[q], run);
                i[q] -= run * di; j[q] -= run * dj;
                err[q] |= (news == 3);
                s[q] = news;
            }
        }
    }
#pragma unroll
    for (int q = 0; q < NP; q++) {
        if (j[q] > 0 && s[q] != OP_I) err[q] |= 1;
        if (i[q] > 0 && s[q] != OP_J) err[q] |= 1;
        while (j[q] > 0) { const int c = j[q] < 32 ? j[q] : 32; C2B_PUSH4(q, OP_I, c); j[q] -= c; }
        while (i[q] > 0) { const int c = i[q] < 32 ? i[q] : 32; C2B_PUSH4(q, OP_J, c); i[q] -= c; }
        if (n[q] & 15) {
            const int ix = n[q] >> 4, used = 2 * (n[q] & 15);
            const uint32_t a = (acc[q] >> (32 - used)) | (~0u << used);
            if (hl == (ix >> 1)) { if (ix & 1) hi[q] = a; else lo[q] = a; }
        }
        out[q].ops = (uint64_t)lo[q] | ((uint64_t)hi[q] << 32); out[q].ops2 = ~0ull; out[q].n = n[q]; out[q].err = err[q];
    }
#undef C2B_PUSH4
}

C2B_DEV int match_count_half(const KParams &P, const RefDev &R, const uint8_t *codes, int J, const Walked &wk)
{
    const int hl = wp::lane() & 15;
    const uint64_t lo = 0x5555555555555555ull;
    int base_i = R.I, base_j = J, match = 0;
#pragma unroll 1
    for (int word = 0; word < 2; word++) {
        const uint64_t ops = word ? wk.ops2 : wk.ops;
        const int ci = 32 - wp::popcll((ops >> 1) & lo);
        const int cj = 32 - wp::popcll(ops & lo);
        int pk = (ci << 16) | cj;
#pragma unroll
        for (int d = 1; d < 16; d <<= 1) { const int v = wp::shfl_up(pk, d); if (hl >= d) pk += v; }
        const int tot = wp::shfl(pk, (wp::lane() & 16) | 15);
        pk -= (ci << 16) | cj;
        int i = base_i - (pk >> 16), j = base_j - (pk & 0xffff);
        uint64_t rest = ops;
#pragma unroll 4
        for (int e = 0; e < 32; e++) {
            const int op = (int)rest & 3;
            rest >>= 2;
            if (op == OP_NONE) continue;
            if (op == OP_M && (uint32_t)P.alpha[codes[j - 1]] == (uint32_t)R.asc[i - 1]) match++;
            i -= (op != OP_I); j -= (op != OP_J);
        }
        base_i -= tot >> 16; base_j -= tot & 0xffff;
    }
#pragma unroll
    for (int d = 8; d >= 1; d >>= 1) match += wp::shfl_xor(match, d);
    return match;
}

C2B_DEV void align_group(const KParams &P, ASmem &S, const uint32_t *staged_prof, int64_t wq, int warp_slot)
{
    const int lane = wp::lane(), g = lane >> 3;
    const int64_t first = 4 * wq;
    const bool multi = P.ref_id == nullptr && P.n_refs > 1;
    bool quad = (P.tbq != nullptr || P.tb != nullptr) && 2 * first + 7 < nreads(P) && (!multi || P.n_refs <= RG_MAX_REFS);
    int r0 = 0;
    uint32_t ringmask = 0;
    if (quad) {
        const int x = lane & 7;
        const int64_t rd = read_at(P, 2 * first + x);
        const int Jx = (int)(P.offsets[rd + 1] - P.offsets[rd]);
        const int rx = P.ref_id ? P.ref_id[rd] : 0;
        r0 = wp::shfl(rx, 0);
        const int Jn = wp::shfl_xor(Jx, 1);
        bool ok = rx == r0 && Jx == Jn && Jx >= 1 && Jx <= RG_COMBO && Jx + 32 <= P.TS;
        const int k0 = multi ? 0 : r0, k1 = multi ? P.n_refs : r0 + 1;
        for (int k = k0; k < k1; k++) {
            const RefDev &R = refdev(P, k);
            ok = ok && !R.coding && Jx <= R.pk_maxJ;
            const bool rk = P.tbq != nullptr && R.rg_ok && R.I + Jx <= PK_MAX_ALN && Jx - R.I <= RG_MAXD && R.I - Jx <= RG_MAXD;
            if (wp::ballot(rk) == 0xffffffffu) ringmask |= 1u << (k - k0);
        }
        quad = wp::ballot(ok) == 0xffffffffu;
        if (!P.tb && ringmask != (k1 - k0 >= 32 ? 0xffffffffu : (1u << (k1 - k0)) - 1u)) quad = false;
    }
    if (!quad) {
#pragma unroll 1
        for (int q = 0; q < 4; q++) {
            if (2 * (first + q) >= nreads(P)) break;
            const int64_t rdA = read_at(P, 2 * (first + q));
            if (2 * (first + q) + 1 < nreads(P)) leftover_pair(P, rdA, read_at(P, 2 * (first + q) + 1));
            else leftover_one(P, rdA);
        }
        return;
    }
    const int k0 = multi ? 0 : r0, k1 = multi ? P.n_refs : r0 + 1;
    uint2 *tbq = P.tbq ? reinterpret_cast<uint2 *>(P.tbq + (int64_t)warp_slot * P.TS * 64) : nullptr;
    uint32_t okmask = 0, modes = 0;
    uint32_t both2[RG_MAX_REFS] = {0, 0, 0, 0};
    int Jg = 0, Jmax = 0;
#pragma unroll 1
    for (int q = 0; q < 4; q++) {
        const int64_t rdA = read_at(P, 2 * (first + q)), rdB = read_at(P, 2 * (first + q) + 1);
        const int J = (int)(P.offsets[rdA + 1] - P.offsets[rdA]);
        bool bad = false;
#pragma unroll 1
        for (int x = 0; x < 2; x++) bad |= load_codes_a(P, S.lut, P.offsets[x ? rdB : rdA], J, S.fw[x], S.rc[x]);
        wp::sync();
        int mAB = 0; bool agree = true;
        uint32_t bothq[RG_MAX_REFS] = {0, 0, 0, 0};
#pragma unroll 1
        for (int k = k0; k < k1; k++) {
            int m = 0;
#pragma unroll 1
            for (int x = 0; x < 2; x++) m |= strand_mode(P, refdev(P, k), S.fw[x], J) << (2 * x);
            if (k == k0) mAB = m;
#pragma unroll
            for (int x = 0; x < 2; x++) {
                const int mk = (m >> (2 * x)) & 3, m0 = (mAB >> (2 * x)) & 3;
                if (mk == 2) bothq[(k - k0) & (RG_MAX_REFS - 1)] |= 1u << x;
                else if (mk != (m0 == 2 ? 0 : m0)) agree = false;
            }
        }
        const int mA = mAB & 3, mB = mAB >> 2;
        if (!bad && agree) {
            const uint8_t *cA = mA == 1 ? S.rc[0] : S.fw[0], *cB = mB == 1 ? S.rc[1] : S.fw[1];
            for (int p = lane; p < J; p += 32) S.combo[q][p] = (uint8_t)(cA[p] * P.nq + cB[p]);
            okmask |= 1u << q; modes |= (uint32_t)mAB << (4 * q);
#pragma unroll
            for (int kk = 0; kk < RG_MAX_REFS; kk++) both2[kk] |= bothq[kk] << (2 * q);
            if (g == q) Jg = J;
            if (J > Jmax) Jmax = J;
        }
        wp::sync();
    }
    uint32_t good2 = 0;
#pragma unroll
    for (int q = 0; q < 4; q++) if ((okmask >> q) & 1u) good2 |= 3u << (2 * q);
    if (!P.tb) {
#pragma unroll
        for (int kk = 0; kk < RG_MAX_REFS; kk++) { good2 &= ~both2[kk]; both2[kk] = 0; }
    }
    int npass = 0, ntried = 0, nboth = 0;
#pragma unroll 1
    for (int k = k0; k < k1 && good2; k++) {
        const RefDev &R = refdev(P, k);
        const uint32_t bothk = both2[(k - k0) & (RG_MAX_REFS - 1)];
        const uint32_t ring2 = good2 & ~bothk;
        nboth += wp::popc(bothk & good2);
        const bool staged = (k == 0 && staged_prof != nullptr);
        uint32_t pass2 = 0;
        if (((ringmask >> (k - k0)) & 1u) && ring2) {
        if (staged) dp_ring<true>(P, R, staged_prof, S.combo[g], Jg, Jmax + R.lstar, tbq, S.fin);
        else dp_ring<false>(P, R, R.prof2, S.combo[g], Jg, Jmax + R.lstar, tbq, S.fin);
        wp::sync();
        const int fl = 3 * ((lane & 24) | (R.lstar & 7));
        const uint32_t cM = Jg > 0 ? S.fin[fl] : PK_SENT, cX = Jg > 0 ? S.fin[fl + 1] : PK_SENT, cY = Jg > 0 ? S.fin[fl + 2] : PK_SENT;
        wp::sync();
        const uint32_t z = wp::max3_2(cM, cY, cX);
        const uint32_t s2 = z & PK_TM;
        const int thr = ring_bound(P, R, Jg) + 512 - P.ge * (R.I + Jg);
        const bool passA = Jg > 0 && (int)((z & 0xffffu) >> 2) > thr, passB = Jg > 0 && (int)(z >> 18) > thr;
        const uint32_t bA = wp::ballot(passA), bB = wp::ballot(passB);
#pragma unroll
        for (int q = 0; q < 4; q++) pass2 |= (((bA >> (8 * q)) & 1u) | (((bB >> (8 * q)) & 1u) << 1)) << (2 * q);
        pass2 &= ring2;
        ntried += wp::popc(ring2);
        {
            int Jq[4], s0[4];
            Walked wk4[4];
            uint32_t walkmask = 0;
#pragma unroll
            for (int q = 0; q < 4; q++) {
                const uint32_t sq = wp::shflu(s2, 8 * q);
                Jq[q] = wp::shfl(Jg, 8 * q);
                s0[q] = (lane & 16) ? (int)(sq >> 16) : (int)(sq & 3u);
                if ((pass2 >> (2 * q)) & 3u) walkmask |= 1u << q;
            }
            walk_ring4(P, R, Jq, tbq, s0, walkmask, wk4);
#pragma unroll
            for (int q = 0; q < 4; q++) {
                if (!((walkmask >> q) & 1u)) continue;
                const Walked &wk = wk4[q];
                const uint32_t eb = wp::ballot(wk.err != 0);
                if (eb & 0xffffu) pass2 &= ~(1u << (2 * q));
                if (eb >> 16) pass2 &= ~(2u << (2 * q));
                const int h = lane >> 4, hl = lane & 15;
                if (!((pass2 >> (2 * q + h)) & 1u)) continue;
                const int64_t rd = read_at(P, 2 * (first + q) + h);
                const int64_t slot = oslot(P, rd, k);
                if (hl < P.NW) P.gops[slot * P.NW + hl] = wk.ops;
                if (hl == 0) {
                    const int mode = (int)((modes >> (4 * q + 2 * h)) & 3u);
                    P.gmeta[slot] = gmeta_pack(wk.n, mode == 1, GM_NONE);
                }
            }
        }
        npass += wp::popc(pass2);
        } else ntried += wp::popc(ring2);
        const uint32_t failed = ring2 & ~pass2;
        if ((failed | (bothk & good2)) && P.tb) {
            uint2 *tb2 = reinterpret_cast<uint2 *>(P.tb + (int64_t)warp_slot * P.tb_words_per_warp);
            int32_t *bnd = P.bnd + (int64_t)warp_slot * P.bnd_words_per_warp;
            const int h = lane >> 4, hl = lane & 15;
#pragma unroll 1
            for (int job = 0; job < 16; job++) {
                const int q = job >> 2, kind = job & 3;
                if (kind == 3) continue;
                const uint32_t fq = (failed >> (2 * q)) & 3u;
                const uint32_t bq = ((bothk & good2) >> (2 * q)) & 3u;
                if (kind == 0 ? fq == 0 : !((bq >> (kind - 1)) & 1u)) continue;
                const int Jp = wp::shfl(Jg, 8 * q);
                const uint8_t *combo = S.combo[q];
                wp::sync();
                if (kind) {
                    const int64_t rdx = read_at(P, 2 * (first + q) + (kind - 1));
                    load_codes_a(P, S.lut, P.offsets[rdx], Jp, S.fw[0], S.rc[0]);
                    wp::sync();
                    for (int p = lane; p < Jp; p += 32) S.fw[1][p] = (uint8_t)(S.fw[0][p] * P.nq + S.rc[0][p]);
                    combo = S.fw[1];
                    wp::sync();
                }
                const Walked wk = align_pair(P, R, staged ? staged_prof : R.prof2, staged, combo, Jp, tb2, nullptr, bnd);
                const uint32_t eb = wp::ballot(wk.err != 0);
                if (kind == 0) {
                    const bool mine = ((fq >> h) & 1u) && !((h ? (eb >> 16) : (eb & 0xffffu)));
                    if (mine) {
                        const int64_t rd = read_at(P, 2 * (first + q) + h);
                        const int64_t slot = oslot(P, rd, k);
                        if (hl < P.NW) P.gops[slot * P.NW + hl] = wk.ops;
                        if (hl + 16 < P.NW) P.gops[slot * P.NW + 16 + hl] = wk.ops2;
                        if (hl == 0) P.gmeta[slot] = gmeta_pack(wk.n, (int)((modes >> (4 * q + 2 * h)) & 3u) == 1, GM_NONE);
                    }
                    const uint32_t mb = wp::ballot(mine);
                    if (mb & 0xffffu) pass2 |= 1u << (2 * q);
                    if (mb >> 16) pass2 |= 2u << (2 * q);
                } else {
                    const int nm = match_count_half(P, R, h ? S.rc[0] : S.fw[0], Jp, wk);
                    const int sc = score_milli(nm, wk.n > 0 ? wk.n : 1);
                    const int sc_fw = wp::shfl(sc, 0), sc_rc = wp::shfl(sc, 16);
                    const int pick = sc_rc > sc_fw ? 1 : 0;
                    const uint32_t bit = 1u << (2 * q + kind - 1);
                    if (eb) good2 &= ~bit;
                    else if (h == pick) {
                        const int64_t rd = read_at(P, 2 * (first + q) + (kind - 1));
                        const int64_t slot = oslot(P, rd, k);
                        if (hl < P.NW) P.gops[slot * P.NW + hl] = wk.ops;
                        if (hl + 16 < P.NW) P.gops[slot * P.NW + 16 + hl] = wk.ops2;
                        if (hl == 0) P.gmeta[slot] = gmeta_pack(wk.n, pick, GM_NONE);
                    }
                }
            }
        }
        pass2 |= bothk & good2;
        good2 &= pass2;
        wp::sync();
    }
#ifndef C2B_EMU
    if (tbq && ringmask) {
        const char *base = reinterpret_cast<const char *>(tbq);
        const int64_t bytes = (int64_t)P.TS * 64 * 4;
        for (int64_t o = (int64_t)lane * 128; o < bytes; o += 32 * 128)
            asm volatile("discard.global.L2 [%0], 128;" ::"l"(base + o) : "memory");
    }
#endif
    if (lane == 0) {
        wp::addg(&P.wb->align_settled, wp::popc(good2));
        wp::addg(&P.wb->ring_kept, npass);
        wp::addg(&P.wb->ring_sent, ntried - npass + nboth + 2 * (k1 - k0) * (4 - wp::popc(okmask)));
    }
#pragma unroll 1
    for (int q = 0; q < 4; q++) {
        const int64_t rdA = read_at(P, 2 * (first + q)), rdB = read_at(P, 2 * (first + q) + 1);
        const uint32_t gq = (good2 >> (2 * q)) & 3u;
        if (gq) {
            const int64_t rd = (lane & 1) ? rdB : rdA;
            const int k = k0 + (lane >> 1);
            if (k < k1 && ((gq >> (lane & 1)) & 1u)) { const int64_t slot = oslot(P, rd, k); P.gmeta[slot] = (P.gmeta[slot] & 0x00ffffffu) | (GM_ALIGNED << 24); }
        }
        if (gq == 0) leftover_pair(P, rdA, rdB);
        else if (gq != 3u) leftover_one(P, gq == 1u ? rdB : rdA);
    }
}

C2B_DEV bool align_narrow16(const KParams &P, ASmem &S, const uint32_t *staged_prof, int64_t w16, int warp_slot)
{
    constexpr int RL = 4, DLO = 4 * RL + 1, DHI = 9 * RL - 4 * RL - 9;
    static_assert(DLO == RN_DLO && DHI == RN_DHI, "the diagonal tier's routing test assumes this band");
    const int lane = wp::lane(), g = lane >> 2;
    const int64_t first = 16 * w16;
    if (!P.left2 || P.tbq == nullptr || first + 15 >= nreads(P) || (P.ref_id == nullptr && P.n_refs > 1)) return false;
    int r0, J0;
    {
        const int64_t rd = read_at(P, first + (lane & 15));
        const int Jx = (int)(P.offsets[rd + 1] - P.offsets[rd]);
        const int rx = P.ref_id ? P.ref_id[rd] : 0;
        r0 = wp::shfl(rx, 0); J0 = wp::shfl(Jx, 0);
        const RefDev &R = refdev(P, r0);
        const bool ok = rx == r0 && Jx == J0 && Jx >= 1 && Jx <= RG_COMBO && Jx + 32 <= P.TS && R.rg_ok && !R.coding && Jx <= R.pk_maxJ &&
                        R.I + Jx <= PK_MAX_ALN && Jx - R.I <= RG_MAXD && R.I - Jx <= RG_MAXD;
        if (wp::ballot(ok) != 0xffffffffu) return false;
    }
    const RefDev &R = refdev(P, r0);
    const int J = J0;
    uint2 *tbq = reinterpret_cast<uint2 *>(P.tbq + (int64_t)warp_slot * P.TS * 64);
    uint32_t modes = 0, use2 = 0;
#pragma unroll 1
    for (int q = 0; q < 8; q++) {
        const int64_t rdA = read_at(P, first + 2 * q), rdB = read_at(P, first + 2 * q + 1);
        bool badA = load_codes_a(P, S.lut, P.offsets[rdA], J, S.fw[0], S.rc[0]);
        bool badB = load_codes_a(P, S.lut, P.offsets[rdB], J, S.fw[1], S.rc[1]);
        wp::sync();
        int m = 0;
#pragma unroll 1
        for (int x = 0; x < 2; x++) m |= strand_mode(P, R, S.fw[x], J) << (2 * x);
        const int mA = m & 3, mB = m >> 2;
        const uint8_t *cA = mA == 1 ? S.rc[0] : S.fw[0], *cB = mB == 1 ? S.rc[1] : S.fw[1];
        for (int p = lane; p < J; p += 32) S.combo[q][p] = (uint8_t)(cA[p] * P.nq + cB[p]);
        modes |= (uint32_t)m << (4 * q);
        if (!badA && mA != 2) use2 |= 1u << (2 * q);
        if (!badB && mB != 2) use2 |= 2u << (2 * q);
        wp::sync();
    }
    const bool staged = (r0 == 0 && staged_prof != nullptr);
    if (staged) dp_ring<true, RL>(P, R, staged_prof, S.combo[g], J, J + R.lstar, tbq, S.fin);
    else dp_ring<false, RL>(P, R, R.prof2, S.combo[g], J, J + R.lstar, tbq, S.fin);
    wp::sync();
    const int fl = 3 * ((lane & ~(RL - 1)) | (R.lstar & (RL - 1)));
    const uint32_t cM = S.fin[fl], cX = S.fin[fl + 1], cY = S.fin[fl + 2];
    wp::sync();
    const uint32_t z = wp::max3_2(cM, cY, cX);
    const uint32_t s2 = z & PK_TM;
    const int thr = ring_bound(P, R, J, DLO, DHI) + 512 - P.ge * (R.I + J);
    const uint32_t bA = wp::ballot((int)((z & 0xffffu) >> 2) > thr), bB = wp::ballot((int)(z >> 18) > thr);
    uint32_t pass2 = 0;
#pragma unroll
    for (int q = 0; q < 8; q++) pass2 |= (((bA >> (RL * q)) & 1u) | (((bB >> (RL * q)) & 1u) << 1)) << (2 * q);
    pass2 &= use2;
#pragma unroll 1
    for (int half = 0; half < 2; half++) {
        const int q0 = 4 * half;
        int Jq[4], s0[4];
        Walked wk4[4];
        uint32_t walkmask = 0;
#pragma unroll
        for (int q = 0; q < 4; q++) {
            const uint32_t sq = wp::shflu(s2, RL * (q0 + q));
            Jq[q] = J;
            s0[q] = (lane & 16) ? (int)(sq >> 16) : (int)(sq & 3u);
            if ((pass2 >> (2 * (q0 + q))) & 3u) walkmask |= 1u << q;
        }
        if (!walkmask) continue;
        walk_ring4<RL, 4>(P, R, Jq, tbq, s0, walkmask, wk4, q0);
#pragma unroll
        for (int q = 0; q < 4; q++) {
            if (!((walkmask >> q) & 1u)) continue;
            const int qq = q0 + q;
            const Walked &wk = wk4[q];
            const uint32_t eb = wp::ballot(wk.err != 0);
            if (eb & 0xffffu) pass2 &= ~(1u << (2 * qq));
            if (eb >> 16) pass2 &= ~(2u << (2 * qq));
            const int h = lane >> 4, hl = lane & 15;
            if (!((pass2 >> (2 * qq + h)) & 1u)) continue;
            const int64_t rd = read_at(P, first + 2 * qq + h);
            const int64_t slot = oslot(P, rd, r0);
            if (hl < P.NW) P.gops[slot * P.NW + hl] = wk.ops;
            if (hl == 0) P.gmeta[slot] = gmeta_pack(wk.n, (int)((modes >> (4 * qq + 2 * h)) & 3u) == 1, GM_ALIGNED);
        }
    }
#ifndef C2B_EMU
    {
        const char *base = reinterpret_cast<const char *>(tbq);
        const int64_t bytes = (int64_t)P.TS * 64 * 4;
        for (int64_t o = (int64_t)lane * 128; o < bytes; o += 32 * 128)
            asm volatile("discard.global.L2 [%0], 128;" ::"l"(base + o) : "memory");
    }
#endif
    const uint32_t rest = 0xffffu & ~pass2;
    if (lane < 16 && ((rest >> lane) & 1u)) {
        const unsigned long long pos = wp::fetch_add(&P.wb->launch.tier2_n, 1ull);
        P.left2[pos] = (int32_t)read_at(P, first + lane);
    }
    if (lane == 0) {
        wp::addg(&P.wb->align_settled, wp::popc(pass2));
        wp::addg(&P.wb->ring_kept, wp::popc(pass2));
        wp::addg(&P.wb->tier2, 16 - wp::popc(pass2));
    }
    return true;
}

C2B_DEV void align_loop(const KParams &P, ASmem &S, const uint32_t *staged_prof, int warp)
{
    const int lane = wp::lane();
    asmem_init(P, S);
    const int64_t nrd = nreads(P);
    const unsigned ahead = (unsigned)wp::grid_warps();
    if (P.left2) {
        const unsigned total = (unsigned)((nrd + 15) / 16);
        for (;;) {
            unsigned w = 0;
            if (lane == 0) w = (unsigned)wp::fetch_work(P.work_counter);
            w = (unsigned)wp::shfl((int)w, 0);
            if (w >= total) break;
            if (w + ahead < total) {
                const int64_t g = (int64_t)w + ahead;
                if (!P.pair_order) {
                    const int64_t last = 16 * g + 16 < nrd ? 16 * g + 16 : nrd;
                    const int64_t a = P.offsets[16 * g] + (int64_t)lane * 128;
                    if (a < P.offsets[last]) wp::prefetch_l2(P.reads + a);
                } else {
                    const int64_t x = 16 * g + (lane >> 1);
                    if (x < nrd) {
                        const int64_t rd = read_at(P, x);
                        const int64_t b1 = P.offsets[rd + 1];
                        for (int64_t a = (P.offsets[rd] & ~(int64_t)127) + (int64_t)(lane & 1) * 128; a < b1; a += 256)
                            wp::prefetch_l2(P.reads + a);
                    }
                }
            }
            if (!align_narrow16(P, S, staged_prof, (int64_t)w, warp)) {
                align_group(P, S, staged_prof, 2 * (int64_t)w, warp);
                wp::sync();
                if (8 * (2 * (int64_t)w + 1) < nrd) align_group(P, S, staged_prof, 2 * (int64_t)w + 1, warp);
            }
            wp::sync();
        }
        return;
    }
    const unsigned total = (unsigned)((nrd + 7) / 8);
    for (;;) {
        unsigned w = 0;
        if (lane == 0) w = (unsigned)wp::fetch_work(P.work_counter);
        w = (unsigned)wp::shfl((int)w, 0);
        if (w >= total) break;
        if (w + ahead < total && !P.pair_order) {
            const int64_t g = (int64_t)w + ahead;
            const int64_t last = 8 * g + 8 < nrd ? 8 * g + 8 : nrd;
            const int64_t a = P.offsets[8 * g] + (int64_t)lane * 128;
            if (a < P.offsets[last]) wp::prefetch_l2(P.reads + a);
        }
        align_group(P, S, staged_prof, (int64_t)w, warp);
        wp::sync();
    }
}

constexpr int B_RD_BYTES = 32 * 16;

static_assert(C2B_NSCAL <= 32, "one lane per scalar slot");
template <int NA> struct ScAcc { long long v[NA]; int ref[NA]; unsigned wmax; };

template <int NA>
C2B_DEV void sc_init(ScAcc<NA> &A)
{
#pragma unroll
    for (int x = 0; x < NA; x++) { A.v[x] = 0; A.ref[x] = -1; }
    A.wmax = 0;
}

template <int NA>
C2B_DEV void sc_acc(ScAcc<NA> &A, const KParams &P, int r, int slot, long long val)
{
    const int lane = wp::lane();
    const int k = NA == 1 ? 0 : (r & (NA - 1));
#pragma unroll
// ... 361 lines not shown
    rec.best_ref = (int16_t)r;
    RowOut o; o.ins_n = o.del_n = o.sub_n = 0; o.n_ins_all = o.n_ins_win = o.n_del_all = o.n_del_win = 0;
    o.n_del_pos = o.n_sub_all = 0; o.nent = 0;
    c2b_edit *ed = P.edits ? P.edits + oslot(P, rd, r) * (int64_t)P.edit_cap : nullptr;
    const bool counted = !ambiguous && (!first || nth == 0) && w > 0;
    const bool len_inline = counted && !two_scans && !ign_i && !ign_d;
    scan(o, ed, RM_SCAL | ((counted && !two_scans) ? RM_VEC : 0) | (len_inline ? RM_LEN : 0));
    const bool has_d = !ign_d && o.del_n > 0, has_i = !ign_i && o.ins_n > 0, has_s = !ign_s && o.sub_n > 0;
    const bool modified = has_d || has_i || has_s;
    uint32_t astatus = 0;
    if (P.edits && o.nent > P.edit_cap) astatus |= C2B_ST_EDIT_OVERFLOW;
    if (counted) {
        const bool discard = two_scans && (o.del_n > 0 || o.ins_n > 0);
        if (discard) sc_acc(A, P, r, C2B_S_DISCARDED, w);
        else {
            const bool entered = modified || R.tem != 0;
            const bool lenv = !len_inline && entered && (o.n_ins_win > 0 || o.n_del_win > 0);
            if (two_scans || lenv) scan(o, nullptr, (two_scans ? RM_VEC : 0) | (lenv ? RM_LEN : 0));
            if (entered) edited_update_acc(A, P, R, r, o, w);
            sc_acc(A, P, r, C2B_S_TOTAL, w);
            sc_acc(A, P, r, modified ? C2B_S_MODIFIED : C2B_S_UNMODIFIED, w);
        }
    } else if (ambiguous && nth == 0 && w > 0) sc_acc(A, P, r, C2B_S_AMBIGUOUS_W, w);
    if (counted && (two_scans || expand)) {
        const bool discarded = two_scans && (o.del_n > 0 || o.ins_n > 0), joined = !ONE && expand && !first && rec.n_winners > 1;
        if (discarded != joined) sc_acc(A, P, r, modified ? C2B_S_CLASS_MODIFIED : C2B_S_CLASS_UNMODIFIED, discarded ? w : -w);
    }
    int irr = 0;
    if (lane == 0) {
        c2b_aln_rec b = multi ? load_aln(P.alns + oslot(P, rd, r)) : a;
        b.insertion_n = (uint16_t)o.ins_n; b.deletion_n = (uint16_t)o.del_n; b.substitution_n = (uint16_t)o.sub_n;
        b.n_ins_all = (uint16_t)o.n_ins_all; b.n_ins_win = (uint16_t)o.n_ins_win;
        b.n_del_all = (uint16_t)o.n_del_all; b.n_del_win = (uint16_t)o.n_del_win;
        b.n_del_pos_all = (uint16_t)o.n_del_pos; b.n_sub_all = (uint16_t)o.n_sub_all;
        b.n_edits = (uint16_t)o.nent; b.modified = modified; b.status |= (uint8_t)astatus;
        irr = b.irregular_ends;
        P.alns[oslot(P, rd, r)] = b;
    }
    irr = wp::shfl(irr, 0);
    rec.status |= astatus;
    const bool is_last = (rec.winner_mask >> (r & 31)) >> 1 == 0;
    if (is_last) {
        const long long total_mods = o.n_ins_all + o.n_del_pos + o.n_sub_all;
        const long long in_win = o.sub_n + o.del_n + o.ins_n;
        sc_acc(A, P, r, C2B_S_N_GLOBAL_SUBS, cnt * o.n_sub_all);
        sc_acc(A, P, r, C2B_S_N_SUBS_OUTSIDE_WINDOW, cnt * (o.n_sub_all - o.sub_n));
        sc_acc(A, P, r, C2B_S_N_MODS_IN_WINDOW, cnt * in_win);
        sc_acc(A, P, r, C2B_S_N_MODS_OUTSIDE_WINDOW, cnt * (total_mods - in_win));
        if (irr) sc_acc(A, P, r, C2B_S_N_READS_IRREGULAR_ENDS, cnt);
        sc_acc(A, P, r, C2B_S_N_ALIGNED_UNIQUE, 1);
        sc_acc(A, P, r, C2B_S_N_ALIGNED_COUNT, cnt);
    }
}

template <bool ONE>
C2B_DEV void classify_read(const KParams &P, int64_t rd, const BPre &pre, const BSmem &S, ScAcc<ONE ? 1 : RG_MAX_REFS> &A)
{
    const int lane = wp::lane();
    const int r_begin = pre.r_begin;
    const int r_end = r_begin + pre.nref;
    const int64_t off = pre.off;
    const int J = pre.J;
    const bool multi = !ONE && (r_end - r_begin) > 1;

    c2b_read_rec rec; rec.winner_mask = 0; rec.best_score_milli = -1000; rec.best_ref = -1; rec.n_winners = 0;
    rec.ambiguous = 0; rec.status = 0;
    ColCtx cx[ONE ? 1 : RG_MAX_REFS];
    c2b_aln_rec a; init_aln(a, 0);
#pragma unroll 1
    for (int r = r_begin; r < r_end; r++) {
        const RefDev &R = refdev(P, r);
        const int64_t slot = oslot(P, rd, r);
        ColCtx &c = cx[ONE ? 0 : r - r_begin];
        const uint32_t gm = pre.gm[ONE ? 0 : r - r_begin];
        c.ops = S.ops[ONE ? 0 : r - r_begin]; c.rd = S.rd + (int)((uintptr_t)(P.reads + off) & 15); c.n = (int)(gm & 0xffffu); c.J = J; c.strand = (int)((gm >> 16) & 1u);
        uint8_t *o_read = P.strings ? P.strings + (slot * 2) * (int64_t)P.W : nullptr;
        const ColOut co = colscan0(P, R, c, o_read, o_read ? o_read + P.W : nullptr);
        note_aln(rec, a, R, r, co, c.n, c.strand, A);
        if (lane == 0 && multi) P.alns[slot] = a;
    }
    if (multi) wp::sync();
    if (rec.best_score_milli <= 0) {
        rec.winner_mask = 0; rec.n_winners = 0;
        if (lane == 0) { if (!multi) P.alns[oslot(P, rd, r_begin)] = a; P.recs[rd] = rec; }
        return;
    }
    const bool expand = P.flags & C2B_F_EXPAND_AMBIGUOUS, first = P.flags & C2B_F_ASSIGN_FIRST;
    const bool ambiguous = !ONE && rec.n_winners > 1 && !first && !expand;
    rec.ambiguous = ambiguous;
    const long long w = pre.qw;
    int nth = 0;
#pragma unroll 1
    for (int r = r_begin; r < r_end; r++) {
        if (!((rec.winner_mask >> (r & 31)) & 1u)) continue;
        const RefDev &R = refdev(P, r);
        const ColCtx &c = cx[ONE ? 0 : r - r_begin];
        classify_winner<ONE>(P, R, rd, r, rec, a, multi, ambiguous, nth, pre.cnt, w, A,
                             [&](RowOut &o, c2b_edit *ed, int mode) { colscan1(P, R, c, o, ed, w, mode); });
        nth++;
    }
    if (!ONE && (P.flags & C2B_F_HDR_REF1) && multi && r_begin == 0 && !ambiguous && w > 0) {
        const uint32_t eff = first ? (rec.winner_mask & (0u - rec.winner_mask)) : rec.winner_mask;
        if (eff != 1u) {
            const RefDev &R0 = P.refs[0];
            RowOut dummy; dummy.ins_n = dummy.del_n = dummy.sub_n = 0; dummy.n_ins_all = dummy.n_ins_win = 0;
            dummy.n_del_all = dummy.n_del_win = dummy.n_del_pos = dummy.n_sub_all = 0; dummy.nent = 0;
            for (int r = 1; r < r_end; r++) {
                if (!((eff >> (r & 31)) & 1u)) continue;
                colscan1(P, R0, cx[0], dummy, nullptr, w, RM_REF1, P.refs[r].vec);
                sc_acc(A, P, r, C2B_S_REF1_W, w);
            }
        }
    }
    if (lane == 0) P.recs[rd] = rec;
}

template <bool ONE>
C2B_DEV void classify_loop(const KParams &P, BSmem &S, int64_t warp, int64_t nwarps)
{
    const int64_t nw = nwarps;
    const int64_t total_bytes = P.offsets[P.n_reads];
    const int64_t n = nreads(P);
    int64_t x = warp;
    if (x >= n) return;
    ScAcc<ONE ? 1 : RG_MAX_REFS> acc;
    sc_init(acc);
    int32_t rd = (int32_t)read_at(P, x), rd1 = 0, rd2 = 0;
    BPreA a1 = classify_pre_a(P, rd);
    BPre pre = classify_pre_b<ONE>(P, rd, a1, total_bytes);
    if (x + nw < n) { rd1 = (int32_t)read_at(P, x + nw); a1 = classify_pre_a(P, rd1); }
    if (x + 2 * nw < n) rd2 = (int32_t)read_at(P, x + 2 * nw);
    while (x < n) {
        const BPre cur = pre;
        const int32_t rc = rd;
        if (cur.go) classify_stage<ONE>(cur, S);
        wp::sync();
        const int64_t nxt = x + nw;
        if (nxt < n) {
            pre = classify_pre_b<ONE>(P, rd1, a1, total_bytes);
            rd = rd1;
            if (nxt + nw < n) { a1 = classify_pre_a(P, rd2); rd1 = rd2; }
            if (nxt + 2 * nw < n) rd2 = (int32_t)read_at(P, nxt + 2 * nw);
        }
        if (cur.go) classify_read<ONE>(P, rc, cur, S, acc);
        wp::sync();
        x = nxt;
    }
    sc_flush(acc, P);
}

constexpr int DG_PROVED = 0, DG_KEEP = 1, DG_ROUTE = 2;
struct DSmem {
    uint4 pl[2][10];
    int32_t pl_ref;
    uint8_t fw[RG_COMBO], rc[RG_COMBO];
    uint8_t lut[256];
    int64_t off[33];
    int32_t ref[32], cnt[32], qw[32];
};

C2B_DEV void diag_classify(const KParams &P, const DSmem &S, const RefDev &R, const uint8_t *c, int64_t rd, int r, int strand,
                           long long cnt, long long w, ScAcc<1> &A)
{
    const int lane = wp::lane(), I = R.I;
    const uint32_t lt = (1u << lane) - 1u;
    const int64_t slot = oslot(P, rd, r);
    const int nsteps = (I + 31) >> 5;
    uint8_t *o_read = P.strings ? P.strings + (slot * 2) * (int64_t)P.W + P.W - I : nullptr;
    int match = 0;
    uint32_t irr = 0, mmis = 0;
#pragma unroll 1
    for (int m = 0; m < nsteps; m++) {
        const int p = 32 * m + lane;
        const bool valid = p < I;
        const uint32_t rdc = valid ? P.alpha[c[p]] : 0u, rfc = valid ? R.asc[p] : 0u;
        const uint32_t Bmis = wp::ballot(valid && rdc != rfc);
        match += wp::popc(wp::ballot(valid && rdc == rfc));
        irr |= wp::ballot(valid && (p == 0 || p == I - 1) && rdc != rfc);
        if (o_read && valid) { o_read[p] = (uint8_t)rdc; o_read[P.W + p] = (uint8_t)rfc; }
        if (lane == m) mmis = Bmis;
    }
    ColOut co; co.n_match = match; co.irregular = irr != 0;
    c2b_read_rec rec; rec.winner_mask = 0; rec.best_score_milli = -1000; rec.best_ref = -1; rec.n_winners = 0;
    rec.ambiguous = 0; rec.status = 0;
    c2b_aln_rec a;
    note_aln(rec, a, R, r, co, I, strand, A);
    if (rec.best_score_milli <= 0) {
        rec.winner_mask = 0; rec.n_winners = 0;
        if (lane == 0) { P.alns[slot] = a; P.recs[rd] = rec; }
        return;
    }
    auto scan = [&](RowOut &o, c2b_edit *ed, int mode) {
        const bool scal = mode & RM_SCAL, vec = mode & RM_VEC, ign_s = P.flags & C2B_F_IGNORE_SUBSTITUTIONS;
        unsigned long long *V = R.vec;
        const int vs = P.vstride;
#pragma unroll 1
        for (int m = 0; m < nsteps; m++) {
            const uint32_t bm = wp::shflu(mmis, m);
            if (!bm) continue;
            const int p = 32 * m + lane;
            const bool differs = (bm >> lane) & 1u;
            const uint32_t rdc = differs ? P.alpha[c[p]] : 0u;
            const bool issub = differs && rdc != 'N';
            const bool inc_p = differs && (R.incl[p] & 1u);
            const int rcode = differs ? S.lut[rdc] : 0;
            if (scal) {
                const uint32_t Bs = wp::ballot(issub), Bsw = wp::ballot(issub && inc_p);
                o.n_sub_all += wp::popc(Bs); o.sub_n += wp::popc(Bsw);
                if (Bs) {
                    const int idx = o.nent + wp::popc(Bs & lt);
                    if (issub && idx < P.edit_cap && ed) {
                        c2b_edit e; e.a = (uint16_t)p; e.b = 0; e.type = 1; e.in_window = inc_p; e.base = (uint8_t)rdc; e.pad = 0;
                        ed[idx] = e;
                    }
                    o.nent += wp::popc(Bs);
                }
            }
            if (vec) {
                if (issub) {
                    wp::addg(V + (int64_t)C2B_V_ALL_SUB * vs + p, w);
                    if (!ign_s) {
                        wp::addg(V + (int64_t)(C2B_V_SUBBASE0 + rcode) * vs + p, w);
                        if (inc_p) wp::addg(V + (int64_t)C2B_V_SUB * vs + p, w);
                    }
                }
                if (differs) {
                    const int rc = R.rcode[p];
                    wp::addg(V + (int64_t)(C2B_V_BASEDEV0 + rcode) * vs + p, w);
                    if (rc != 255) wp::addg(V + (int64_t)(C2B_V_BASEDEV0 + rc) * vs + p, -w);
                }
            }
        }
    };
    classify_winner<true>(P, R, rd, r, rec, a, false, false, 0, cnt, w, A, scan);
    if (lane == 0) P.recs[rd] = rec;
}

C2B_DEV int route_read(const KParams &P, DSmem &S, const RefDev &R, int r, const uint8_t *c, int D)
{
    if (!R.rt_ok || D > R.rt_thr) return DG_KEEP;
    const int lane = wp::lane(), I = R.I, nb = (I + 31) >> 5;
    auto match = [](uint4 a, uint4 b) { return ~((a.x ^ b.x) | (a.y ^ b.y)) & a.z & b.z; };
    auto shifted = [](uint4 lo, uint4 hi, int t) {
        return make_uint4(wp::funnel_r(lo.x, hi.x, t), wp::funnel_r(lo.y, hi.y, t), wp::funnel_r(lo.z, hi.z, t), 0u);
    };
    auto below = [](int n) -> uint32_t { return n >= 32 ? ~0u : n <= 0 ? 0u : (1u << n) - 1u; };
    for (int b = 0; b < nb; b++) {
        const int x = 32 * b + lane, q = x < I ? c[x] : 255;
        const uint32_t p0 = wp::ballot(q & 1), p1 = wp::ballot(q & 2), v = wp::ballot(q < 4);
        if (lane == 0) S.pl[0][b] = make_uint4(p0, p1, v, 0u);
    }
    if (lane < 2) S.pl[0][nb + lane] = make_uint4(0u, 0u, 0u, 0u);
    const bool fresh = S.pl_ref != r;
    wp::sync();
    if (fresh) {
        if (lane < nb + 2) S.pl[1][lane] = R.rt_pl[lane];
        if (lane == 0) S.pl_ref = r;
    }
    wp::sync();
    const int s = lane - 16, t = s < 0 ? -s : s, cs = R.rt_c[lane];
    const uint4 *Ap = S.pl[s < 0 ? 0 : 1], *Bp = S.pl[s < 0 ? 1 : 0];
    int run = 0, best = RT_OFF, bb = 1, mst = 0;
#pragma unroll 1
    for (int b = 0; b < nb; b++) {
        const uint32_t m0 = match(S.pl[0][b], S.pl[1][b]) & below(I - t - 32 * b);
        const uint32_t ms = match(Ap[b], shifted(Bp[b], Bp[b + 1], t));
        const int k = wp::popc(ms);
        run += wp::popc(m0) - k; mst += k;
        if (run > best) { best = run; bb = b + 1; }
    }
    const int val = cs == RT_OFF ? RT_OFF : R.rt_mx * (mst + best) + cs;
    int vmax = val;
#pragma unroll
    for (int d = 16; d >= 1; d >>= 1) { const int o = wp::shfl_xor(vmax, d); if (o > vmax) vmax = o; }
    if (vmax == RT_OFF) return DG_ROUTE;
    const int L = wp::ffs(wp::ballot(val == vmax)) - 1;
    const int s1 = L - 16, t1 = s1 < 0 ? -s1 : s1, w0 = wp::shfl(bb, L) - 1, F1 = wp::shfl(mst + best, L), c1 = wp::shfl(cs, L);
    const uint4 *A1 = S.pl[s1 < 0 ? 0 : 1], *B1 = S.pl[s1 < 0 ? 1 : 0];
    uint32_t m0w[2], msw[2];
#pragma unroll
    for (int h = 0; h < 2; h++) {
        m0w[h] = match(S.pl[0][w0 + h], S.pl[1][w0 + h]) & below(I - t1 - 32 * (w0 + h));
        msw[h] = match(A1[w0 + h], shifted(B1[w0 + h], B1[w0 + h + 1], t1));
    }
    const int F0 = F1 - (wp::popc(m0w[0]) - wp::popc(msw[0]));
    const uint32_t a = lane < 16 ? m0w[0] : m0w[1], bm = lane < 16 ? msw[0] : msw[1];
    const int j = (2 * lane) & 31;
    const int e0 = (int)((a >> j) & 1u) - (int)((bm >> j) & 1u), e1 = (int)((a >> (j + 1)) & 1u) - (int)((bm >> (j + 1)) & 1u);
    int incl = e0 + e1;
#pragma unroll
    for (int d = 1; d < 32; d <<= 1) { const int v = wp::shfl_up(incl, d); if (lane >= d) incl += v; }
    const int imul = s1 < 0 ? 1 : t1;
    int e = RT_OFF;
    auto cand = [&](int p, int F) {
        if (p >= 1 && p <= I - t1) { const int v = R.rt_mx * F + imul * (R.g4[p] >> 2) + c1; if (v > e) e = v; }
    };
    const int pa = 32 * w0 + 2 * lane + 1;
    cand(pa, F0 + incl - e1);
    cand(pa + 1, F0 + incl);
    if (lane == 0) cand(32 * w0, F0);
#pragma unroll
    for (int d = 16; d >= 1; d >>= 1) { const int o = wp::shfl_xor(e, d); if (o > e) e = o; }
    return e > R.rt_thr ? DG_KEEP : DG_ROUTE;
}

C2B_DEV int diag_read(const KParams &P, DSmem &S, int64_t rd, int64_t off, int J, int r, long long cnt, long long w, ScAcc<1> &A)
{
    const int lane = wp::lane();
    const RefDev &R = refdev(P, r);
    const int I = R.I;
    if (!R.dg_ok || J != I || J > RG_COMBO || J + 32 > P.TS || J > R.pk_maxJ || I + J > PK_MAX_ALN) return DG_KEEP;
    const bool bad = load_codes_a(P, S.lut, off, J, S.fw, S.rc);
    wp::sync();
    if (bad) return P.route ? DG_ROUTE : DG_KEEP;
    const int mode = strand_mode(P, R, S.fw, J);
    if (mode == 2) return P.route ? DG_ROUTE : DG_KEEP;
    const uint8_t *c = mode == 1 ? S.rc : S.fw;
    const int32_t *prof = R.prof;
    const int Ipad = R.Ipad, dS = R.dg_S;
    int acc[9];
#pragma unroll
    for (int s = 0; s < 9; s++) acc[s] = 0;
    for (int k = lane; k < I; k += 32) {
        const int32_t *pk = prof + k;
#pragma unroll
        for (int s = -4; s <= 4; s++) {
            const int j = k + s;
            if ((s < 0 ? -s : s) <= dS && j >= 0 && j < J) acc[s + 4] += pk[(int)c[j] * Ipad];
        }
    }
#pragma unroll
    for (int s = 0; s < 9; s++)
#pragma unroll
        for (int d = 16; d >= 1; d >>= 1) acc[s] += wp::shfl_xor(acc[s], d);
    bool proved = acc[4] > R.dg_thr4;
#pragma unroll
    for (int s = -4; s <= 4; s++)
        if (s != 0 && (s < 0 ? -s : s) <= dS) proved = proved && acc[4] > acc[s + 4] + R.dg_c4[s + 4];
    if (!proved) return P.route == 0 ? DG_KEEP : P.route == 2 ? DG_ROUTE : route_read(P, S, R, r, c, acc[4] >> 2);
    const int64_t slot = oslot(P, rd, r);
    if (lane < 16 && lane < P.NW) {
        const int rem = I - 32 * lane;
        P.gops[slot * P.NW + lane] = rem >= 32 ? 0ull : rem <= 0 ? ~0ull : (~0ull << (2 * rem));
    }
    if (lane == 0) P.gmeta[slot] = gmeta_pack(I, mode == 1, GM_ALIGNED);
    diag_classify(P, S, R, c, rd, r, mode == 1, cnt, w, A);
    return DG_PROVED;
}

C2B_DEV void dsmem_init(const KParams &P, DSmem &S)
{
    for (int k = wp::lane(); k < 256; k += 32) S.lut[k] = P.lut[k];
    if (wp::lane() == 0) S.pl_ref = -1;
    wp::sync();
}

C2B_DEV void list_append(int32_t *list, unsigned long long *n, uint32_t mask, int64_t first)
{
    if (!mask) return;
    const int lane = wp::lane();
    unsigned long long pos = 0;
    if (lane == 0) pos = wp::fetch_add(n, (unsigned long long)wp::popc(mask));
    pos = (unsigned long long)(uint32_t)wp::shfl((int)(uint32_t)pos, 0) | ((unsigned long long)(uint32_t)wp::shfl((int)(uint32_t)(pos >> 32), 0) << 32);
    if ((mask >> lane) & 1u) list[pos + wp::popc(mask & ((1u << lane) - 1u))] = (int32_t)(first + lane);
}

C2B_DEV int diag_unit(const KParams &P, DSmem &S, int64_t u, ScAcc<1> &A, int &routed)
{
    const int lane = wp::lane();
    const int64_t first = 32 * u;
    const int n = P.n_reads - first < 32 ? (int)(P.n_reads - first) : 32;
    {
        const int64_t rd = first + lane;
        if (lane < n) {
            S.off[lane] = P.offsets[rd]; S.ref[lane] = P.ref_id ? P.ref_id[rd] : 0;
            S.cnt[lane] = P.count ? P.count[rd] : 1; S.qw[lane] = P.qweight ? P.qweight[rd] : S.cnt[lane];
        }
        if (lane == 0) S.off[n] = P.offsets[first + n];
    }
    wp::sync();
#ifndef C2B_EMU
    {
        const int64_t b0 = S.off[0] & ~(int64_t)127, b1 = S.off[n];
        for (int64_t a = b0 + (int64_t)lane * 128; a < b1; a += 32 * 128) asm volatile("prefetch.global.L2 [%0];" ::"l"(P.reads + a));
    }
#endif
    uint32_t fail = 0, route = 0;
#pragma unroll 1
    for (int x = 0; x < n; x++) {
        const int64_t off = S.off[x];
        const int v = diag_read(P, S, first + x, off, (int)(S.off[x + 1] - off), S.ref[x], S.cnt[x], S.qw[x], A);
        if (v != DG_PROVED) fail |= 1u << x;
        if (v == DG_ROUTE) route |= 1u << x;
        wp::sync();
    }
    list_append(P.left0, &P.wb->launch.diag_n, fail, first);
    if (P.route) {
        list_append(P.left1, &P.wb->launch.narrow_n, fail & ~route, first);
        list_append(P.left2, &P.wb->launch.tier2_n, route, first);
    }
    routed = wp::popc(route);
    return n - wp::popc(fail);
}

C2B_DEV void diag_loop(const KParams &P, DSmem &S, int64_t warp, int64_t nwarps)
{
    dsmem_init(P, S);
    ScAcc<1> acc;
    sc_init(acc);
    const int64_t units = (P.n_reads + 31) / 32;
    int proved = 0, seen = 0, routed = 0;
    for (int64_t u = warp; u < units; u += nwarps) {
        int k = 0;
        proved += diag_unit(P, S, u, acc, k);
        routed += k;
        seen += P.n_reads - 32 * u < 32 ? (int)(P.n_reads - 32 * u) : 32;
        wp::sync();
    }
    sc_flush(acc, P);
    if (wp::lane() == 0 && seen) {
        WorkBlock &wb = *P.wb;
        wp::addg(&wb.diag_proved, proved); wp::addg(&wb.diag_listed, seen - proved);
        wp::addg(&wb.tier2, routed);
        wp::addg(&wb.routed, routed); wp::addg(&wb.kept, seen - proved - routed);
    }
}

}
```

### crispresso2_b200/engine.py

```python
import ctypes as C

import numpy as np

from . import _lib

_DNA_COMP = {"A": "T", "C": "G", "G": "C", "T": "A"}


class EngineError(RuntimeError):
    pass


class BatchResult:

    def __init__(self, recs, alns, strings, edits, W, ops=None, meta=None, engine=None, buf=None, off=None, ref_id=None):
        self.recs, self.alns, self.strings, self.edits, self.W = recs, alns, strings, edits, W
        self.ops, self.meta, self._engine, self._buf, self._off, self._ref_id = ops, meta, engine, buf, off, ref_id

    def strings_block(self, lo, hi):
        if self.strings is not None:
            return self.strings[lo:hi]
        e = self._engine
        off = np.ascontiguousarray(self._off[lo:hi + 1])
        rid = None if self._ref_id is None else np.ascontiguousarray(self._ref_id[lo:hi], dtype=np.int32)
# ... 85 lines not shown
            rc = (C.c_char_p * max(ns, 1))(*[s.encode() for s in ref.get("rc_seeds", [])[:ns]])
            arr[k].seq, arr[k].len = sb, len(sb)
            arr[k].gap_incentive, arr[k].include_idx, arr[k].n_include = gi.ctypes.data, inc.ctypes.data, len(inc)
            arr[k].min_aln_score = float(ref.get("min_aln_score", 0))
            arr[k].score_rows = rows.ctypes.data
            arr[k].fw_seeds, arr[k].rc_seeds, arr[k].n_seeds = fw, rc, ns
            arr[k].tot_exon_len_mod = int(sum(ref.get("exon_len_mods", []) or []))
            cmask = None
            if ref.get("contains_coding_seq", False):
                cmask = np.zeros(len(sb), dtype=np.uint8)
                ex = np.asarray(sorted(set(ref.get("exon_positions", []))), dtype=np.int64)
                sp = np.asarray(sorted(set(ref.get("splicing_positions", []))), dtype=np.int64)
                cmask[ex[(ex >= 0) & (ex < len(sb))]] |= 1
                cmask[sp[(sp >= 0) & (sp < len(sb))]] |= 2
                arr[k].coding_mask = cmask.ctypes.data
            keep.append((sb, gi, inc, rows, fw, rc, cmask))
        self._check(self.L.c2b_configure(self.h, C.byref(p), len(ref_names), arr), "c2b_configure")
        self.n_refs, self.alphabet, self.edit_cap = len(ref_names), alphabet, int(edit_cap)
        self.ref_names = list(ref_names)
        self.ref_lens = [len(refs[n]["sequence"]) for n in ref_names]
        self.ref_seqs = [refs[n]["sequence"] for n in ref_names]
        self.flags = int(flags)
        return self

    def set_edit_cap(self, cap):
        self._check(self.L.c2b_set_edit_cap(self.h, int(cap)), "c2b_set_edit_cap")
        self.edit_cap = int(cap)

    def string_width(self, max_read_len):
        w = self.L.c2b_string_width(self.h, int(max_read_len))
        if w < 0:
            raise EngineError("engine not configured")
        return w

    def _max_len_of(self, W):
        return max(1, W - max(self.ref_lens))

    def align_packed(self, buf, off, count=None, qweight=None, ref_id=None, strings=True, edits=True, compact=False, on_launch=None):
        n = len(off) - 1
        maxj = int(np.max(np.diff(off))) if n else 1
        W = self.string_width(max(maxj, 1))
        nr = 1 if ref_id is not None else self.n_refs
        recs = np.zeros(n, dtype=_lib.REC_DTYPE)
        alns = np.zeros((n, nr), dtype=_lib.ALN_DTYPE)
        earr = np.zeros((n, nr, self.edit_cap), dtype=_lib.EDIT_DTYPE) if (edits and self.edit_cap) else None

        def ptr(a):
            return None if a is None else a.ctypes.data

        buf = np.ascontiguousarray(buf, dtype=np.uint8)
        off = np.ascontiguousarray(off, dtype=np.int64)
        cnt = None if count is None else np.ascontiguousarray(count, dtype=np.int32)
        qw = None if qweight is None else np.ascontiguousarray(qweight, dtype=np.int32)
        rid = None if ref_id is None else np.ascontiguousarray(ref_id, dtype=np.int32)
        if compact:
            ops = np.zeros((n, nr, W // 32), dtype=np.uint64)
            meta = np.zeros((n, nr), dtype=np.uint32)
            if on_launch is not None:
                on_launch()
            self._check(self.L.c2b_align_batch_compact(self.h, ptr(buf) if len(buf) else None, ptr(off), n, ptr(cnt), ptr(qw),
                                                       ptr(rid), ptr(recs), ptr(alns), ptr(ops), ptr(meta), ptr(earr)),
                        "c2b_align_batch_compact")
            return BatchResult(recs, alns, None, earr, W, ops=ops, meta=meta, engine=self, buf=buf, off=off, ref_id=rid)
        sarr = np.zeros((n, nr, 2, W), dtype=np.uint8) if strings else None
        self._check(self.L.c2b_align_batch(self.h, ptr(buf) if len(buf) else None, ptr(off), n, ptr(cnt), ptr(qw),
                                           ptr(rid), ptr(recs), ptr(alns), ptr(sarr), ptr(earr)), "c2b_align_batch")
        return BatchResult(recs, alns, sarr, earr, W)

    def align(self, reads, **kw):
        buf, off = pack_reads(reads)
        return self.align_packed(buf, off, **kw)

    def classify_pair(self, read_al, ref_al, include_idx, alphabet=None, legacy=False):
        n = len(ref_al)
        if alphabet is None:
            extra = sorted(set(read_al) - set("ACGTN-"))
            alphabet = "ACGTN" + "".join(extra)
        inc = np.ascontiguousarray(include_idx, dtype=np.int64)
        aln = np.zeros(1, dtype=_lib.ALN_DTYPE)
        edits = np.zeros(n + 1, dtype=_lib.EDIT_DTYPE)
        rc = self.L.c2b_classify_aligned_flags(self.h, read_al.encode(), ref_al.encode(), n, alphabet.encode(), len(alphabet),
                                               inc.ctypes.data, len(inc), _lib.F_LEGACY_INS if legacy else 0, aln.ctypes.data,
                                               edits.ctypes.data)
        self.n_refs = 0
        if rc == -2:
            raise NotImplementedError("aligned pair outside the aligner's invariants: %s"
                                      % self.L.c2b_last_error(self.h).decode())
        self._check(rc, "c2b_classify_aligned")
        if aln[0]["status"]:
            raise EngineError("c2b_classify_aligned: status %d" % aln[0]["status"])
        return aln[0], edits

    def counts_layout(self):
        a, b, c, d = C.c_int32(), C.c_int32(), C.c_int32(), C.c_int32()
        self._check(self.L.c2b_counts_layout(self.h, C.byref(a), C.byref(b), C.byref(c), C.byref(d)), "c2b_counts_layout")
        return a.value, b.value, c.value, d.value

    def counts_reset(self):
        self._check(self.L.c2b_counts_reset(self.h), "c2b_counts_reset")

    def hist_layout(self):
        a, b, c = C.c_int32(), C.c_int32(), C.c_int32()
        self._check(self.L.c2b_counts_hist_layout(self.h, C.byref(a), C.byref(b), C.byref(c)), "c2b_counts_hist_layout")
        return a.value, b.value, c.value

    def counts_raw(self):
        nr, nv, st, ns = self.counts_layout()
        nh, hs, _ = self.hist_layout()
        out = np.zeros(nr * (nv * st + nh * hs + ns), dtype=np.int64)
        self._check(self.L.c2b_counts_read(self.h, out.ctypes.data, out.size), "c2b_counts_read")
        return out

    def counts_device(self):
        p, n = C.c_void_p(), C.c_size_t()
        self._check(self.L.c2b_counts_device(self.h, C.byref(p), C.byref(n)), "c2b_counts_device")
        return p.value, n.value

    def counts(self, raw=None):
        from .counts import CountBlock
        nr, nv, st, ns = self.counts_layout()
        raw = self.counts_raw() if raw is None else np.asarray(raw, dtype=np.int64)
        nh, hs, hz = self.hist_layout()
        return CountBlock(raw, self.ref_names, self.ref_seqs, self.alphabet, nv, st, ns, nh, hs, hz, self.flags)

    def sync(self):
        self._check(self.L.c2b_sync(self.h), "c2b_sync")

    def last_kernel_ms(self):
        return float(self.L.c2b_last_kernel_ms(self.h))

    def path_counts(self):
        a, b = C.c_int64(), C.c_int64()
        self._check(self.L.c2b_path_counts(self.h, C.byref(a), C.byref(b)), "c2b_path_counts")
        return a.value, b.value

    def band_reruns(self):
        return int(self.L.c2b_band_reruns(self.h))

    def ring_counts(self):
        a, b = C.c_int64(0), C.c_int64(0)
        self.L.c2b_ring_counts(self.h, C.byref(a), C.byref(b))
        return a.value, b.value

    def diag_counts(self):
        a, b, c = C.c_int64(0), C.c_int64(0), C.c_int64(0)
        self._check(self.L.c2b_diag_counts(self.h, C.byref(a), C.byref(b), C.byref(c)), "c2b_diag_counts")
        return a.value, b.value, c.value

    def route_counts(self):
        a, b = C.c_int64(0), C.c_int64(0)
        self._check(self.L.c2b_route_counts(self.h, C.byref(a), C.byref(b)), "c2b_route_counts")
        return a.value, b.value

    def launch_count(self):
        return int(self.L.c2b_launch_count(self.h))
```

### include/c2b200.h

```cpp
#ifndef C2B200_H
#define C2B200_H
#include <stddef.h>
#include <stdint.h>

#ifdef __cplusplus
extern "C" {
#endif

#define C2B_MAX_Q        8
#define C2B_MAX_SEEDS    8
#define C2B_MAX_SEED_LEN 20
#define C2B_MAX_REF_LEN  1024
#define C2B_MAX_READ_LEN 512
#define C2B_MAX_ALN_LEN  1024
#define C2B_MAX_REFS     32
#define C2B_MAX_POOLED_REFS 1024

#define C2B_OK            0
#define C2B_E_CUDA       -1
#define C2B_E_ARG        -2
#define C2B_E_LIMIT      -3
#define C2B_E_STATE      -4

#define C2B_F_IGNORE_SUBSTITUTIONS  1u
#define C2B_F_IGNORE_INSERTIONS     2u
#define C2B_F_IGNORE_DELETIONS      4u
#define C2B_F_EXPAND_AMBIGUOUS      8u
#define C2B_F_ASSIGN_FIRST         16u
#define C2B_F_DISCARD_INDEL_READS  32u
#define C2B_F_NO_STRAND_SEARCH     64u
#define C2B_F_NO_PAIRING          128u
#define C2B_F_LEGACY_INS         1024u
#define C2B_F_NO_RING             512u
#define C2B_F_HDR_REF1            256u

typedef struct {
    int32_t  gap_open;
    int32_t  gap_extend;
    int32_t  seed_count;
    int32_t  seed_min;
    uint32_t flags;
    int32_t  nq;
    char     alphabet[C2B_MAX_Q];
    uint8_t  complement[C2B_MAX_Q];
    int32_t  edit_cap;
} c2b_params;

typedef struct {
    const char    *seq;
    int32_t        len;
    const int64_t *gap_incentive;
    const int64_t *include_idx;
    int32_t        n_include;
    double         min_aln_score;
    const int64_t *score_rows;
    const char *const *fw_seeds;
    const char *const *rc_seeds;
    int32_t        n_seeds;
    int32_t        tot_exon_len_mod;
    const uint8_t *coding_mask;
} c2b_ref;

typedef struct {
    uint16_t n_match;
    uint16_t aln_len;
    int32_t  score_milli;
    uint8_t  strand;
    uint8_t  status;
    uint16_t n_edits;
    uint16_t insertion_n, deletion_n, substitution_n;
    uint16_t n_ins_all, n_ins_win;
    uint16_t n_del_all, n_del_win;
    uint16_t n_del_pos_all;
    uint16_t n_sub_all;
    uint8_t  irregular_ends;
    uint8_t  modified;
} c2b_aln_rec;

#define C2B_ST_BAD_CHAR       1u
#define C2B_ST_UNDEFINED      2u
#define C2B_ST_EDIT_OVERFLOW  4u
#define C2B_ST_TOO_LONG       8u

typedef struct {
    uint32_t winner_mask;
    int32_t  best_score_milli;
    int16_t  best_ref;
    uint8_t  n_winners;
    uint8_t  ambiguous;
    uint32_t status;
} c2b_read_rec;

typedef struct {
    uint16_t a;
    uint16_t b;
    uint8_t  type;
    uint8_t  in_window;
    uint8_t  base;
    uint8_t  pad;
} c2b_edit;

enum {
    C2B_V_ALL_INS = 0, C2B_V_ALL_INS_LEFT, C2B_V_ALL_DEL, C2B_V_ALL_SUB,
    C2B_V_INS, C2B_V_DEL, C2B_V_SUB,
    C2B_V_SUBBASE0,
    C2B_V_BASEDEV0 = C2B_V_SUBBASE0 + C2B_MAX_Q,
    C2B_V_INS_LEN = C2B_V_BASEDEV0 + C2B_MAX_Q + 1,
    C2B_V_DEL_LEN,
    C2B_V_R1_ALL_INS, C2B_V_R1_ALL_INS_LEFT, C2B_V_R1_ALL_DEL, C2B_V_R1_ALL_SUB,
    C2B_V_R1_BASEDEV0,
    C2B_V_INS_NONCODING = C2B_V_R1_BASEDEV0 + C2B_MAX_Q + 1, C2B_V_DEL_NONCODING, C2B_V_SUB_NONCODING,
    C2B_NVEC
};
enum {
    C2B_H_INS_N = 0,
    C2B_H_DEL_N,
    C2B_H_SUB_N,
    C2B_H_EFF_LEN,
    C2B_H_INFRAME,
    C2B_H_FRAMESHIFT,
    C2B_NHIST
};
enum {
    C2B_S_TOTAL = 0, C2B_S_MODIFIED, C2B_S_UNMODIFIED, C2B_S_DISCARDED,
    C2B_S_INS, C2B_S_DEL, C2B_S_SUB,
    C2B_S_ONLY_INS, C2B_S_ONLY_DEL, C2B_S_ONLY_SUB, C2B_S_INS_DEL, C2B_S_INS_SUB, C2B_S_DEL_SUB, C2B_S_INS_DEL_SUB,
    C2B_S_AMBIGUOUS_W,
    C2B_S_N_GLOBAL_SUBS, C2B_S_N_SUBS_OUTSIDE_WINDOW, C2B_S_N_MODS_IN_WINDOW, C2B_S_N_MODS_OUTSIDE_WINDOW,
    C2B_S_N_READS_IRREGULAR_ENDS, C2B_S_N_ALIGNED_UNIQUE, C2B_S_N_ALIGNED_COUNT,
    C2B_S_REF1_W,
    C2B_S_CLASS_MODIFIED, C2B_S_CLASS_UNMODIFIED,
    C2B_S_MOD_FRAMESHIFT, C2B_S_MOD_NON_FRAMESHIFT, C2B_S_NON_MOD_NON_FRAMESHIFT, C2B_S_SPLICING_MODIFIED,
    C2B_NSCAL
};

typedef struct c2b_engine c2b_engine;

int  c2b_create(int device, c2b_engine **out);
void c2b_destroy(c2b_engine *e);
const char *c2b_last_error(const c2b_engine *e);

int  c2b_configure(c2b_engine *e, const c2b_params *p, int32_t n_refs, const c2b_ref *refs);

int  c2b_set_edit_cap(c2b_engine *e, int32_t edit_cap);

int  c2b_string_width(const c2b_engine *e, int32_t max_read_len);

int  c2b_align_batch(c2b_engine *e, const uint8_t *reads, const int64_t *offsets, int64_t n_reads,
                     const int32_t *count, const int32_t *qweight, const int32_t *ref_id,
                     c2b_read_rec *recs, c2b_aln_rec *alns, uint8_t *strings, c2b_edit *edits);

int  c2b_align_batch_compact(c2b_engine *e, const uint8_t *reads, const int64_t *offsets, int64_t n_reads,
                             const int32_t *count, const int32_t *qweight, const int32_t *ref_id,
                             c2b_read_rec *recs, c2b_aln_rec *alns, uint64_t *ops, uint32_t *meta, c2b_edit *edits);
int  c2b_ops_words(const c2b_engine *e, int32_t max_read_len);
int  c2b_expand_alignment(const c2b_engine *e, const uint64_t *ops, uint32_t meta, const char *read, int32_t read_len,
                          const char *ref, int32_t ref_len, char *out_read, char *out_ref);
int  c2b_expand_batch(const c2b_engine *e, const uint8_t *reads, const int64_t *offsets, int64_t n_reads, const int32_t *ref_id,
                      const uint64_t *ops, const uint32_t *meta, int32_t max_read_len, uint8_t *strings, int32_t n_threads);

int  c2b_align_batch_device(c2b_engine *e, const uint8_t *d_reads, const int64_t *d_offsets, int64_t n_reads,
                            int32_t max_read_len, const int32_t *d_count, const int32_t *d_qweight,
                            const int32_t *d_ref_id, c2b_read_rec *d_recs, c2b_aln_rec *d_alns,
                            uint8_t *d_strings, c2b_edit *d_edits);
int  c2b_set_pair_order(c2b_engine *e, const int32_t *d_order);
int  c2b_ops_device(c2b_engine *e, void **d_ops, void **d_meta);
int  c2b_sync(c2b_engine *e);
void *c2b_stream(c2b_engine *e);
double c2b_last_kernel_ms(c2b_engine *e);
int64_t c2b_launch_count(const c2b_engine *e);
int  c2b_path_counts(c2b_engine *e, int64_t *pair_items, int64_t *single_items);
int64_t c2b_band_reruns(c2b_engine *e);
int  c2b_ring_counts(c2b_engine *e, int64_t *ring_pairs, int64_t *ring_fallbacks);
int  c2b_diag_counts(c2b_engine *e, int64_t *proved, int64_t *tier1, int64_t *tier2);
int  c2b_route_counts(c2b_engine *e, int64_t *routed, int64_t *kept);

int  c2b_counts_layout(const c2b_engine *e, int32_t *n_refs, int32_t *n_vec, int32_t *stride, int32_t *n_scal);
int  c2b_counts_hist_layout(const c2b_engine *e, int32_t *n_hist, int32_t *hstride, int32_t *hist_zero);
int  c2b_counts_reset(c2b_engine *e);
int  c2b_counts_read(c2b_engine *e, int64_t *out, size_t n_int64);
int  c2b_counts_device(c2b_engine *e, void **d_ptr, size_t *n_int64);

int  c2b_global_align(c2b_engine *e, const char *read, int32_t read_len, const char *ref, int32_t ref_len,
                      const char *alphabet, int32_t nq, const int64_t *score_rows, const int64_t *gap_incentive,
                      int32_t gap_open, int32_t gap_extend,
                      char *out_read, char *out_ref, int32_t *aln_len, int32_t *n_match);

int  c2b_classify_aligned(c2b_engine *e, const char *read_al, const char *ref_al, int32_t n_cols,
                          const char *alphabet, int32_t nq, const int64_t *include_idx, int32_t n_include,
                          c2b_aln_rec *out, c2b_edit *edits);
int  c2b_classify_aligned_flags(c2b_engine *e, const char *read_al, const char *ref_al, int32_t n_cols,
                                const char *alphabet, int32_t nq, const int64_t *include_idx, int32_t n_include,
                                uint32_t flags, c2b_aln_rec *out, c2b_edit *edits);

typedef struct c2b_fastq c2b_fastq;
int  c2b_fastq_dedup(const char *path, int32_t n_threads, c2b_fastq **out);
int  c2b_fastq_dedup_buffer(const uint8_t *data, size_t n_bytes, int32_t n_threads, c2b_fastq **out);
int64_t c2b_fastq_n_reads(const c2b_fastq *f);
int64_t c2b_fastq_n_unique(const c2b_fastq *f);
int32_t c2b_fastq_max_len(const c2b_fastq *f);
const uint8_t *c2b_fastq_seqs(const c2b_fastq *f);
const int64_t *c2b_fastq_offsets(const c2b_fastq *f);
const int32_t *c2b_fastq_counts(const c2b_fastq *f);
const int64_t *c2b_fastq_first_index(const c2b_fastq *f);
void c2b_fastq_free(c2b_fastq *f);
const char *c2b_fastq_last_error(void);
int  c2b_fastq_gpu_available(void);
int  c2b_fastq_dedup_gpu(const char *path, int32_t device, c2b_fastq **out);
int  c2b_fastq_dedup_gpu_buffer(const uint8_t *data, size_t n_bytes, int32_t device, c2b_fastq **out);
int  c2b_sam_dedup_gpu_buffer(const uint8_t *data, size_t n_bytes, int32_t device, c2b_fastq **out);
int  c2b_sam_dedup_buffer(const uint8_t *data, size_t n_bytes, int32_t n_threads, c2b_fastq **out);

int  c2b_rc_merge_weights(const uint8_t *seqs, const int64_t *offsets, int64_t n, const int32_t *counts,
                          const uint8_t *member, int32_t *weights, int32_t n_threads);

int64_t c2b_screen_reads(const uint8_t *seqs, const int64_t *offsets, int64_t n, int32_t max_len, uint8_t *out, int32_t n_threads);

int  c2b_serial_stats(const c2b_read_rec *recs, const c2b_aln_rec *alns, const int32_t *counts, int64_t n, int32_t nr,
                      int64_t *out, uint8_t *aligned, int32_t n_threads);

int  c2b_fastq_filter(const char *path_in, const char *path_out, int32_t min_bp_qual_in_read, int32_t min_av_read_qual,
                      int32_t min_bp_qual_or_N, int32_t n_threads, int64_t *n_in, int64_t *n_out);

typedef struct c2b_alleles c2b_alleles;
int  c2b_alleles_build(const uint8_t *reads, const int64_t *offsets, const uint64_t *ops, const uint32_t *meta, int32_t NW,
                       int64_t n_rows, const int64_t *row_read, const int64_t *row_slot, const int32_t *row_ref,
                       const int64_t *row_count, int32_t n_refs, const char *const *ref_seqs, const int32_t *ref_lens,
                       const uint8_t *comp256, int32_t n_threads, c2b_alleles **out);
void c2b_alleles_free(c2b_alleles *a);
int64_t        c2b_alleles_n(const c2b_alleles *a);
const int64_t *c2b_alleles_order(const c2b_alleles *a);
const uint8_t *c2b_alleles_arena(const c2b_alleles *a);
const int64_t *c2b_alleles_offsets(const c2b_alleles *a);
const int32_t *c2b_alleles_lengths(const c2b_alleles *a);
int  c2b_alleles_write_tsv(const c2b_alleles *a, const char *path, int64_t n_sel, const int64_t *rows,
                           const int32_t *name_id, const char *const *names, const int32_t *status_id, const char *const *statuses,
                           const int32_t *n_deleted, const int32_t *n_inserted, const int32_t *n_mutated,
                           const int32_t *pct_id, const char *const *pcts, int32_t n_threads);
int64_t c2b_alleles_around_cut(c2b_alleles *a, int64_t n_sel, const int64_t *rows, int32_t cut_point, int32_t plot_left,
                               int32_t plot_right, const uint8_t *unedited, const int32_t *n_deleted, const int32_t *n_inserted,
                               const int32_t *n_mutated, const double *pct);
int32_t c2b_alleles_cut_width(const c2b_alleles *a);
int  c2b_alleles_cut_fetch(const c2b_alleles *a, uint8_t *seq, uint8_t *ref, int32_t *wlen, uint8_t *unedited, int32_t *n_deleted,
                           int32_t *n_inserted, int32_t *n_mutated, int64_t *reads, double *pct);

#define C2B_ANN_SAM_OPTIONAL  (1u << 16)
typedef struct c2b_annotation c2b_annotation;
int  c2b_annotate_build(c2b_engine *e, const uint8_t *reads, const int64_t *offsets, int64_t n_unique, const int32_t *bidx,
                        int32_t R, int32_t NW, int32_t edit_cap, const c2b_read_rec *recs, const c2b_aln_rec *alns,
                        const uint64_t *ops, const uint32_t *meta, const c2b_edit *edits,
                        const uint32_t *amask, const int16_t *aname, const int32_t *label,
                        int32_t n_names, const char *const *names, const uint8_t *name_rev,
                        int32_t n_labels, const char *const *labels,
                        const char *const *ref_seqs, const int32_t *ref_lens, const uint8_t *comp256, uint32_t flags,
                        int64_t chunk, c2b_annotation **out);
void c2b_annotate_free(c2b_annotation *a);
int64_t        c2b_annotate_n(const c2b_annotation *a);
const uint8_t *c2b_annotate_arena(const c2b_annotation *a);
const int64_t *c2b_annotate_offsets(const c2b_annotation *a);
const uint8_t *c2b_annotate_cigar_arena(const c2b_annotation *a);
const int64_t *c2b_annotate_cigar_offsets(const c2b_annotation *a);
const uint8_t *c2b_annotate_flags(const c2b_annotation *a);
const int32_t *c2b_annotate_mapq(const c2b_annotation *a);
const int16_t *c2b_annotate_first(const c2b_annotation *a);
const int64_t *c2b_annotate_last_record(const c2b_annotation *a);
const uint8_t *c2b_annotate_record_arena(const c2b_annotation *a);
const int64_t *c2b_annotate_record_offsets(const c2b_annotation *a);
int  c2b_annotate_write_fastq(const c2b_annotation *a, const uint8_t *seqs, const int64_t *offsets, int64_t n_unique,
                              const char *in_path, const char *out_path, int32_t n_threads);
int  c2b_annotate_write_sam(c2b_annotation *a, const uint8_t *seqs, const int64_t *offsets, int64_t n_unique,
                            const char *in_path, const char *sam_path, const char *header, int32_t n_names,
                            const char *const *chr, const char *const *pos, const uint8_t *rev, int32_t n_threads);
int  c2b_annotate_write_sam_passthrough(const c2b_annotation *a, const uint8_t *seqs, const int64_t *offsets, int64_t n_unique,
                                        const uint8_t *text, size_t n_bytes, const char *sam_path, int32_t n_threads);

int  c2b_fastq_filter_pair(const char *path1_in, const char *path2_in, const char *path1_out, const char *path2_out,
                           int32_t min_bp_qual_in_read, int32_t min_av_read_qual, int32_t min_bp_qual_or_N,
                           int32_t n_threads, int64_t *n_in, int64_t *n_out);

int  c2b_consensus_from_pairs(const char *aln_seq_r1, int32_t ns1, const char *aln_ref_r1, int32_t n1, double score_r1, const char *qual_r1, int32_t nq1,
                              const char *aln_seq_r2, int32_t ns2, const char *aln_ref_r2, int32_t n2, double score_r2, const char *qual_r2, int32_t nq2,
                              char *out_aln, char *out_qual, char *out_ref, int32_t cap,
                              int32_t *n_cols, int32_t *n_qual, int32_t *n_match, int32_t *caching_is_ok);

void *c2b_host_alloc(size_t n_bytes);
void  c2b_host_free(void *p);

#ifdef __cplusplus
}
#endif
#endif
```

Baseline: 82.84 million.

## Score diagonal proof with bit-plane popcounts and prefetch reads via cp.async

```diff
diff --git a/crispresso2_b200/_lib.py b/crispresso2_b200/_lib.py
--- a/crispresso2_b200/_lib.py
+++ b/crispresso2_b200/_lib.py
@@ -74,7 +74,7 @@
 
 EXPORTS = ["c2b_create", "c2b_destroy", "c2b_last_error", "c2b_configure", "c2b_set_edit_cap", "c2b_string_width", "c2b_align_batch",
            "c2b_align_batch_compact", "c2b_ops_words", "c2b_expand_alignment", "c2b_expand_batch", "c2b_ops_device",
-           "c2b_align_batch_device", "c2b_set_pair_order", "c2b_sync", "c2b_stream", "c2b_last_kernel_ms", "c2b_launch_count", "c2b_path_counts", "c2b_band_reruns", "c2b_ring_counts", "c2b_diag_counts", "c2b_route_counts",
+           "c2b_align_batch_device", "c2b_set_pair_order", "c2b_sync", "c2b_stream", "c2b_last_kernel_ms", "c2b_launch_count", "c2b_path_counts", "c2b_band_reruns", "c2b_ring_counts", "c2b_diag_counts", "c2b_route_counts", "c2b_diag_popcount_reads",
            "c2b_counts_layout", "c2b_counts_hist_layout", "c2b_counts_reset", "c2b_counts_read", "c2b_counts_device", "c2b_global_align",
            "c2b_classify_aligned", "c2b_classify_aligned_flags", "c2b_host_alloc", "c2b_host_free",
            "c2b_fastq_dedup", "c2b_fastq_dedup_buffer", "c2b_fastq_gpu_available", "c2b_fastq_dedup_gpu", "c2b_fastq_dedup_gpu_buffer", "c2b_sam_dedup_gpu_buffer", "c2b_sam_dedup_buffer", "c2b_fastq_n_reads", "c2b_fastq_n_unique", "c2b_fastq_max_len",
@@ -149,6 +149,8 @@
     L.c2b_diag_counts.argtypes = [vp, C.POINTER(i64), C.POINTER(i64), C.POINTER(i64)]
     L.c2b_route_counts.restype = C.c_int
     L.c2b_route_counts.argtypes = [vp, C.POINTER(i64), C.POINTER(i64)]
+    L.c2b_diag_popcount_reads.restype = C.c_int
+    L.c2b_diag_popcount_reads.argtypes = [vp, C.POINTER(i64)]
     L.c2b_counts_layout.restype = C.c_int
     L.c2b_counts_layout.argtypes = [vp, C.POINTER(i32), C.POINTER(i32), C.POINTER(i32), C.POINTER(i32)]
     L.c2b_counts_hist_layout.restype = C.c_int
diff --git a/crispresso2_b200/csrc/c2b_core.cuh b/crispresso2_b200/csrc/c2b_core.cuh
--- a/crispresso2_b200/csrc/c2b_core.cuh
+++ b/crispresso2_b200/csrc/c2b_core.cuh
@@ -35,6 +35,9 @@
 C2B_DEV int grid_warps() { return (int)(gridDim.x * (blockDim.x >> 5)); }
 C2B_DEV uint32_t smem_addr(const void *p) { return (uint32_t)__cvta_generic_to_shared(p); }
 C2B_DEV uint32_t lds_u8(uint32_t a) { uint32_t v; asm volatile("ld.shared.u8 %0, [%1];" : "=r"(v) : "r"(a)); return v; }
+C2B_DEV void cp_async16(void *dst, const void *src)
+{ asm volatile("cp.async.ca.shared.global [%0], [%1], 16;" ::"r"(smem_addr(dst)), "l"(__cvta_generic_to_global(src)) : "memory"); }
+C2B_DEV void wait_async() { asm volatile("cp.async.wait_all;" ::: "memory"); }
 C2B_DEV uint4 lds_v4(uint32_t a) { uint4 v; asm volatile("ld.shared.v4.u32 {%0,%1,%2,%3}, [%4];" : "=r"(v.x), "=r"(v.y), "=r"(v.z), "=r"(v.w) : "r"(a)); return v; }
 C2B_DEV uint2 ldcg2(const uint2 *p) { return __ldcg(p); }
 C2B_DEV uint32_t funnel_r(uint32_t lo, uint32_t hi, int sh) { return __funnelshift_r(lo, hi, sh); }
@@ -62,6 +65,8 @@
 #include "warp_emu.h"
 namespace wp {
 C2B_DEV int grid_warps() { return 1; }
+C2B_DEV void cp_async16(void *dst, const void *src) { memcpy(dst, src, 16); }
+C2B_DEV void wait_async() {}
 }
 #endif
 
@@ -97,6 +102,7 @@
     int32_t rg_ok, rg_smax, rg_gmax, rg_gsum;
     int32_t dg_ok, dg_S, dg_thr4;
     int32_t dg_c4[2 * 4 + 1];
+    int32_t dg_two, dg_a4, dg_b4;
     int32_t rt_ok, rt_thr;
     int32_t rt_mx;
     int32_t rt_c[32];
@@ -108,6 +114,7 @@
 struct WorkBlock {
     unsigned long long pair_items, single_items, band_reruns, ring_kept, ring_sent, align_settled;
     unsigned long long diag_proved, diag_listed, tier2, routed, kept;
+    unsigned long long diag_popc;
     struct Launch {
         unsigned long long align_next, tier2_next, general_next;
         unsigned long long widest;
diff --git a/crispresso2_b200/csrc/c2b_engine.cu b/crispresso2_b200/csrc/c2b_engine.cu
--- a/crispresso2_b200/csrc/c2b_engine.cu
+++ b/crispresso2_b200/csrc/c2b_engine.cu
@@ -591,6 +591,20 @@
                 d.dg_c4[s + 4] = (int32_t)(4 * (s == 0 ? 0 : 2 * ge * t + gi0 + (s > 0 ? rf.gap_incentive[I - std::min<int64_t>(t, I)] : t * gI)));
             }
             if (!d.dg_ok) { d.dg_S = 0; d.dg_thr4 = 0; }
+            const int nq4 = std::min(p->nq, 4);
+            int64_t a = 0, b = 0;
+            bool two = d.dg_ok && I <= 256, have_b = false;
+            for (int i = 0; i < I && two; i++) {
+                if (rcode[i] >= nq4) { two = false; break; }
+                for (int q = 0; q < nq4; q++) {
+                    const int64_t v = rf.score_rows[(size_t)q * I + i];
+                    if (q == rcode[i]) { if (i == 0) a = v; else if (v != a) two = false; }
+                    else if (!have_b) { b = v; have_b = true; }
+                    else if (v != b) two = false;
+                }
+            }
+            two = two && 4 * (std::abs(a) + std::abs(b)) * I < (1ll << 30);
+            d.dg_two = two; d.dg_a4 = two ? (int32_t)(4 * a) : 0; d.dg_b4 = two ? (int32_t)(4 * b) : 0;
         }
         {
             const int nq4 = std::min(p->nq, 4);
@@ -989,6 +1003,16 @@
     if (proved) *proved = (int64_t)v.diag_proved;
     if (tier1) *tier1 = (int64_t)v.diag_listed;
     if (tier2) *tier2 = (int64_t)v.tier2;
+    return C2B_OK;
+}
+
+int c2b_diag_popcount_reads(c2b_engine *e, int64_t *reads)
+{
+    if (!e || !e->work.p) return fail(e, C2B_E_STATE, "c2b_diag_popcount_reads: nothing launched yet");
+    WorkBlock v;
+    RTCHK(rt_d2h(&v, e->work.p, sizeof v, e->stream));
+    RTCHK(rt_sync(e->stream));
+    if (reads) *reads = (int64_t)v.diag_popc;
     return C2B_OK;
 }
 
diff --git a/crispresso2_b200/csrc/c2b_split.cuh b/crispresso2_b200/csrc/c2b_split.cuh
--- a/crispresso2_b200/csrc/c2b_split.cuh
+++ b/crispresso2_b200/csrc/c2b_split.cuh
@@ -36,14 +36,14 @@
     if (wp::lane() == 0) { const unsigned long long pos = wp::fetch_add(&P.wb->launch.left_n, 1ull); P.left[pos] = (int32_t)rd; }
 }
 
-C2B_DEV bool load_codes_a(const KParams &P, const uint8_t *lut, int64_t off, int J, uint8_t *fw, uint8_t *rc)
+C2B_DEV bool load_codes_a(const KParams &P, const uint8_t *lut, const uint8_t *src, int J, uint8_t *fw, uint8_t *rc)
 {
     const int lane = wp::lane();
     bool bad = false;
     for (int base = 0; base < J; base += 128) {
         uint8_t ch[4];
 #pragma unroll
-        for (int e = 0; e < 4; e++) { const int p = base + lane + 32 * e; ch[e] = p < J ? P.reads[off + p] : (uint8_t)P.alpha[0]; }
+        for (int e = 0; e < 4; e++) { const int p = base + lane + 32 * e; ch[e] = p < J ? src[p] : (uint8_t)P.alpha[0]; }
 #pragma unroll
         for (int e = 0; e < 4; e++) {
             const int p = base + lane + 32 * e;
@@ -218,7 +218,7 @@
         const int J = (int)(P.offsets[rdA + 1] - P.offsets[rdA]);
         bool bad = false;
 #pragma unroll 1
-        for (int x = 0; x < 2; x++) bad |= load_codes_a(P, S.lut, P.offsets[x ? rdB : rdA], J, S.fw[x], S.rc[x]);
+        for (int x = 0; x < 2; x++) bad |= load_codes_a(P, S.lut, P.reads + P.offsets[x ? rdB : rdA], J, S.fw[x], S.rc[x]);
         wp::sync();
         int mAB = 0; bool agree = true;
         uint32_t bothq[RG_MAX_REFS] = {0, 0, 0, 0};
@@ -328,7 +328,7 @@
                 wp::sync();
                 if (kind) {
                     const int64_t rdx = read_at(P, 2 * (first + q) + (kind - 1));
-                    load_codes_a(P, S.lut, P.offsets[rdx], Jp, S.fw[0], S.rc[0]);
+                    load_codes_a(P, S.lut, P.reads + P.offsets[rdx], Jp, S.fw[0], S.rc[0]);
                     wp::sync();
                     for (int p = lane; p < Jp; p += 32) S.fw[1][p] = (uint8_t)(S.fw[0][p] * P.nq + S.rc[0][p]);
                     combo = S.fw[1];
@@ -421,8 +421,8 @@
 #pragma unroll 1
     for (int q = 0; q < 8; q++) {
         const int64_t rdA = read_at(P, first + 2 * q), rdB = read_at(P, first + 2 * q + 1);
-        bool badA = load_codes_a(P, S.lut, P.offsets[rdA], J, S.fw[0], S.rc[0]);
-        bool badB = load_codes_a(P, S.lut, P.offsets[rdB], J, S.fw[1], S.rc[1]);
+        bool badA = load_codes_a(P, S.lut, P.reads + P.offsets[rdA], J, S.fw[0], S.rc[0]);
+        bool badB = load_codes_a(P, S.lut, P.reads + P.offsets[rdB], J, S.fw[1], S.rc[1]);
         wp::sync();
         int m = 0;
 #pragma unroll 1
@@ -1090,15 +1090,25 @@
 constexpr int DG_PROVED = 0, DG_KEEP = 1, DG_ROUTE = 2;
 struct DSmem {
     uint4 pl[2][10];
+    uint8_t raw[2][RG_COMBO + 32];
     int32_t pl_ref;
     uint8_t fw[RG_COMBO], rc[RG_COMBO];
     uint8_t lut[256];
     int64_t off[33];
+    int64_t total_bytes;
     int32_t ref[32], cnt[32], qw[32];
+    int32_t npop;
 };
 
+C2B_DEV uint32_t pl_match(uint4 a, uint4 b) { return ~((a.x ^ b.x) | (a.y ^ b.y)) & a.z & b.z; }
+C2B_DEV uint4 pl_shifted(uint4 lo, uint4 hi, int t)
+{
+    return make_uint4(wp::funnel_r(lo.x, hi.x, t), wp::funnel_r(lo.y, hi.y, t), wp::funnel_r(lo.z, hi.z, t), 0u);
+}
+C2B_DEV uint32_t pl_below(int n) { return n >= 32 ? ~0u : n <= 0 ? 0u : (1u << n) - 1u; }
+
 C2B_DEV void diag_classify(const KParams &P, const DSmem &S, const RefDev &R, const uint8_t *c, int64_t rd, int r, int strand,
-                           long long cnt, long long w, ScAcc<1> &A)
+                           long long cnt, long long w, ScAcc<1> &A, bool planes)
 {
     const int lane = wp::lane(), I = R.I;
     const uint32_t lt = (1u << lane) - 1u;
@@ -1107,16 +1117,31 @@
     uint8_t *o_read = P.strings ? P.strings + (slot * 2) * (int64_t)P.W + P.W - I : nullptr;
     int match = 0;
     uint32_t irr = 0, mmis = 0;
-#pragma unroll 1
-    for (int m = 0; m < nsteps; m++) {
-        const int p = 32 * m + lane;
-        const bool valid = p < I;
-        const uint32_t rdc = valid ? P.alpha[c[p]] : 0u, rfc = valid ? R.asc[p] : 0u;
-        const uint32_t Bmis = wp::ballot(valid && rdc != rfc);
-        match += wp::popc(wp::ballot(valid && rdc == rfc));
-        irr |= wp::ballot(valid && (p == 0 || p == I - 1) && rdc != rfc);
-        if (o_read && valid) { o_read[p] = (uint8_t)rdc; o_read[P.W + p] = (uint8_t)rfc; }
-        if (lane == m) mmis = Bmis;
+    if (planes) {
+        mmis = lane < nsteps ? ~pl_match(S.pl[0][lane], S.pl[1][lane]) & pl_below(I - 32 * lane) : 0u;
+        int k = wp::popc(mmis);
+#pragma unroll
+        for (int d = 16; d >= 1; d >>= 1) k += wp::shfl_xor(k, d);
+        match = I - k;
+        irr = (wp::shflu(mmis, 0) & 1u) | ((wp::shflu(mmis, nsteps - 1) >> ((I - 1) & 31)) & 1u);
+        if (o_read)
+#pragma unroll 4
+            for (int m = 0; m < nsteps; m++) {
+                const int p = 32 * m + lane;
+                if (p < I) { o_read[p] = (uint8_t)P.alpha[c[p]]; o_read[P.W + p] = R.asc[p]; }
+            }
+    } else {
+#pragma unroll 1
+        for (int m = 0; m < nsteps; m++) {
+            const int p = 32 * m + lane;
+            const bool valid = p < I;
+            const uint32_t rdc = valid ? P.alpha[c[p]] : 0u, rfc = valid ? R.asc[p] : 0u;
+            const uint32_t Bmis = wp::ballot(valid && rdc != rfc);
+            match += wp::popc(wp::ballot(valid && rdc == rfc));
+            irr |= wp::ballot(valid && (p == 0 || p == I - 1) && rdc != rfc);
+            if (o_read && valid) { o_read[p] = (uint8_t)rdc; o_read[P.W + p] = (uint8_t)rfc; }
+            if (lane == m) mmis = Bmis;
+        }
     }
     ColOut co; co.n_match = match; co.irregular = irr != 0;
     c2b_read_rec rec; rec.winner_mask = 0; rec.best_score_milli = -1000; rec.best_ref = -1; rec.n_winners = 0;
@@ -1174,35 +1199,17 @@
     if (lane == 0) P.recs[rd] = rec;
 }
 
-C2B_DEV int route_read(const KParams &P, DSmem &S, const RefDev &R, int r, const uint8_t *c, int D)
+C2B_DEV int route_read(const RefDev &R, const DSmem &S, int D)
 {
     if (!R.rt_ok || D > R.rt_thr) return DG_KEEP;
     const int lane = wp::lane(), I = R.I, nb = (I + 31) >> 5;
-    auto match = [](uint4 a, uint4 b) { return ~((a.x ^ b.x) | (a.y ^ b.y)) & a.z & b.z; };
-    auto shifted = [](uint4 lo, uint4 hi, int t) {
-        return make_uint4(wp::funnel_r(lo.x, hi.x, t), wp::funnel_r(lo.y, hi.y, t), wp::funnel_r(lo.z, hi.z, t), 0u);
-    };
-    auto below = [](int n) -> uint32_t { return n >= 32 ? ~0u : n <= 0 ? 0u : (1u << n) - 1u; };
-    for (int b = 0; b < nb; b++) {
-        const int x = 32 * b + lane, q = x < I ? c[x] : 255;
-        const uint32_t p0 = wp::ballot(q & 1), p1 = wp::ballot(q & 2), v = wp::ballot(q < 4);
-        if (lane == 0) S.pl[0][b] = make_uint4(p0, p1, v, 0u);
-    }
-    if (lane < 2) S.pl[0][nb + lane] = make_uint4(0u, 0u, 0u, 0u);
-    const bool fresh = S.pl_ref != r;
-    wp::sync();
-    if (fresh) {
-        if (lane < nb + 2) S.pl[1][lane] = R.rt_pl[lane];
-        if (lane == 0) S.pl_ref = r;
-    }
-    wp::sync();
     const int s = lane - 16, t = s < 0 ? -s : s, cs = R.rt_c[lane];
     const uint4 *Ap = S.pl[s < 0 ? 0 : 1], *Bp = S.pl[s < 0 ? 1 : 0];
     int run = 0, best = RT_OFF, bb = 1, mst = 0;
 #pragma unroll 1
     for (int b = 0; b < nb; b++) {
-        const uint32_t m0 = match(S.pl[0][b], S.pl[1][b]) & below(I - t - 32 * b);
-        const uint32_t ms = match(Ap[b], shifted(Bp[b], Bp[b + 1], t));
+        const uint32_t m0 = pl_match(S.pl[0][b], S.pl[1][b]) & pl_below(I - t - 32 * b);
+        const uint32_t ms = pl_match(Ap[b], pl_shifted(Bp[b], Bp[b + 1], t));
         const int k = wp::popc(ms);
         run += wp::popc(m0) - k; mst += k;
         if (run > best) { best = run; bb = b + 1; }
@@ -1218,8 +1225,8 @@
     uint32_t m0w[2], msw[2];
 #pragma unroll
     for (int h = 0; h < 2; h++) {
-        m0w[h] = match(S.pl[0][w0 + h], S.pl[1][w0 + h]) & below(I - t1 - 32 * (w0 + h));
-        msw[h] = match(A1[w0 + h], shifted(B1[w0 + h], B1[w0 + h + 1], t1));
+        m0w[h] = pl_match(S.pl[0][w0 + h], S.pl[1][w0 + h]) & pl_below(I - t1 - 32 * (w0 + h));
+        msw[h] = pl_match(A1[w0 + h], pl_shifted(B1[w0 + h], B1[w0 + h + 1], t1));
     }
     const int F0 = F1 - (wp::popc(m0w[0]) - wp::popc(msw[0]));
     const uint32_t a = lane < 16 ? m0w[0] : m0w[1], bm = lane < 16 ? msw[0] : msw[1];
@@ -1242,55 +1249,114 @@
     return e > R.rt_thr ? DG_KEEP : DG_ROUTE;
 }
 
-C2B_DEV int diag_read(const KParams &P, DSmem &S, int64_t rd, int64_t off, int J, int r, long long cnt, long long w, ScAcc<1> &A)
+C2B_DEV int diag_read(const KParams &P, DSmem &S, int64_t rd, const uint8_t *bytes, int J, int r, long long cnt, long long w,
+                      ScAcc<1> &A)
 {
     const int lane = wp::lane();
     const RefDev &R = refdev(P, r);
     const int I = R.I;
     if (!R.dg_ok || J != I || J > RG_COMBO || J + 32 > P.TS || J > R.pk_maxJ || I + J > PK_MAX_ALN) return DG_KEEP;
-    const bool bad = load_codes_a(P, S.lut, off, J, S.fw, S.rc);
+    const bool bad = load_codes_a(P, S.lut, bytes, J, S.fw, S.rc);
     wp::sync();
     if (bad) return P.route ? DG_ROUTE : DG_KEEP;
     const int mode = strand_mode(P, R, S.fw, J);
     if (mode == 2) return P.route ? DG_ROUTE : DG_KEEP;
     const uint8_t *c = mode == 1 ? S.rc : S.fw;
-    const int32_t *prof = R.prof;
-    const int Ipad = R.Ipad, dS = R.dg_S;
-    int acc[9];
-#pragma unroll
-    for (int s = 0; s < 9; s++) acc[s] = 0;
-    for (int k = lane; k < I; k += 32) {
-        const int32_t *pk = prof + k;
-#pragma unroll
-        for (int s = -4; s <= 4; s++) {
-            const int j = k + s;
-            if ((s < 0 ? -s : s) <= dS && j >= 0 && j < J) acc[s + 4] += pk[(int)c[j] * Ipad];
-        }
-    }
-#pragma unroll
-    for (int s = 0; s < 9; s++)
-#pragma unroll
-        for (int d = 16; d >= 1; d >>= 1) acc[s] += wp::shfl_xor(acc[s], d);
-    bool proved = acc[4] > R.dg_thr4;
-#pragma unroll
-    for (int s = -4; s <= 4; s++)
-        if (s != 0 && (s < 0 ? -s : s) <= dS) proved = proved && acc[4] > acc[s + 4] + R.dg_c4[s + 4];
-    if (!proved) return P.route == 0 ? DG_KEEP : P.route == 2 ? DG_ROUTE : route_read(P, S, R, r, c, acc[4] >> 2);
+    const int nb = (I + 31) >> 5, dS = R.dg_S;
+    uint4 rp = make_uint4(0u, 0u, 0u, 0u);
+    bool acgt = false;
+    if (R.dg_two || R.rt_ok) {
+        for (int b = 0; b < nb; b++) {
+            const int x = 32 * b + lane, q = x < I ? c[x] : 255;
+            const uint32_t p0 = wp::ballot(q & 1), p1 = wp::ballot(q & 2), v = wp::ballot(q < 4);
+            if (lane == b) rp = make_uint4(p0, p1, v, 0u);
+        }
+        acgt = wp::ballot(lane < nb && rp.z != pl_below(I - 32 * lane)) == 0;
+        if (lane < nb + 2) S.pl[0][lane] = rp;
+        const bool fresh = S.pl_ref != r;
+        wp::sync();
+        if (fresh) {
+            if (lane < nb + 2) S.pl[1][lane] = R.rt_pl[lane];
+            if (lane == 0) S.pl_ref = r;
+        }
+        wp::sync();
+    }
+    int D;
+    bool proved;
+    if (R.dg_two && acgt) {
+        if (lane == 0) S.npop++;
+        const uint4 z4 = make_uint4(0u, 0u, 0u, 0u);
+        const uint4 rf = lane < nb ? S.pl[1][lane] : z4, rf1 = lane < nb ? S.pl[1][lane + 1] : z4, rp1 = lane < nb ? S.pl[0][lane + 1] : z4;
+        auto total = [](int v) {
+#pragma unroll
+            for (int d = 4; d >= 1; d >>= 1) v += wp::shfl_xor(v, d);
+            return wp::shfl(v, 0);
+        };
+        const int m0 = total(wp::popc(pl_match(rp, rf)));
+        D = R.dg_a4 * m0 + R.dg_b4 * (I - m0);
+        proved = D > R.dg_thr4;
+#pragma unroll
+        for (int t = 1; t <= 4; t++) {
+            if (t > dS) break;
+            const int m = total((wp::popc(pl_match(rf, pl_shifted(rp, rp1, t))) << 16) | wp::popc(pl_match(rp, pl_shifted(rf, rf1, t))));
+            const int mp = m >> 16, mn = m & 0xffff;
+            proved = proved && D > R.dg_a4 * mp + R.dg_b4 * (I - t - mp) + R.dg_c4[4 + t] &&
+                     D > R.dg_a4 * mn + R.dg_b4 * (I - t - mn) + R.dg_c4[4 - t];
+        }
+    } else {
+        const int32_t *prof = R.prof;
+        const int Ipad = R.Ipad;
+        int acc[9];
+#pragma unroll
+        for (int s = 0; s < 9; s++) acc[s] = 0;
+        for (int k = lane; k < I; k += 32) {
+            const int32_t *pk = prof + k;
+#pragma unroll
+            for (int s = -4; s <= 4; s++) {
+                const int j = k + s;
+                if ((s < 0 ? -s : s) <= dS && j >= 0 && j < J) acc[s + 4] += pk[(int)c[j] * Ipad];
+            }
+        }
+#pragma unroll
+        for (int s = 0; s < 9; s++)
+            if ((s < 4 ? 4 - s : s - 4) <= dS)
+#pragma unroll
+                for (int d = 16; d >= 1; d >>= 1) acc[s] += wp::shfl_xor(acc[s], d);
+        D = acc[4];
+        proved = D > R.dg_thr4;
+#pragma unroll
+        for (int s = -4; s <= 4; s++)
+            if (s != 0 && (s < 0 ? -s : s) <= dS) proved = proved && D > acc[s + 4] + R.dg_c4[s + 4];
+    }
+    if (!proved) return P.route == 0 ? DG_KEEP : P.route == 2 ? DG_ROUTE : route_read(R, S, D >> 2);
     const int64_t slot = oslot(P, rd, r);
     if (lane < 16 && lane < P.NW) {
         const int rem = I - 32 * lane;
         P.gops[slot * P.NW + lane] = rem >= 32 ? 0ull : rem <= 0 ? ~0ull : (~0ull << (2 * rem));
     }
     if (lane == 0) P.gmeta[slot] = gmeta_pack(I, mode == 1, GM_ALIGNED);
-    diag_classify(P, S, R, c, rd, r, mode == 1, cnt, w, A);
+    diag_classify(P, S, R, c, rd, r, mode == 1, cnt, w, A, R.dg_two && acgt);
     return DG_PROVED;
 }
 
 C2B_DEV void dsmem_init(const KParams &P, DSmem &S)
 {
     for (int k = wp::lane(); k < 256; k += 32) S.lut[k] = P.lut[k];
-    if (wp::lane() == 0) S.pl_ref = -1;
+    if (wp::lane() == 0) { S.pl_ref = -1; S.npop = 0; }
     wp::sync();
+}
+
+C2B_DEV void diag_stage(const KParams &P, DSmem &S, int x, int b)
+{
+    const int64_t off = S.off[x];
+    if (S.off[x + 1] - off > RG_COMBO) return;
+    const uint8_t *p0 = P.reads + off, *end = P.reads + S.off[x + 1], *lim = P.reads + S.total_bytes;
+    const int lane = wp::lane();
+    const uint8_t *wa = p0 - ((uintptr_t)p0 & 15) + 16 * lane;
+    uint8_t *dst = S.raw[b] + 16 * lane;
+    if (wa >= end) return;
+    if (wa >= P.reads && wa + 16 <= lim) wp::cp_async16(dst, wa);
+    else for (int k = 0; k < 16; k++) if (wa + k >= P.reads && wa + k < lim) dst[k] = wa[k];
 }
 
 C2B_DEV void list_append(int32_t *list, unsigned long long *n, uint32_t mask, int64_t first)
@@ -1314,7 +1380,7 @@
             S.off[lane] = P.offsets[rd]; S.ref[lane] = P.ref_id ? P.ref_id[rd] : 0;
             S.cnt[lane] = P.count ? P.count[rd] : 1; S.qw[lane] = P.qweight ? P.qweight[rd] : S.cnt[lane];
         }
-        if (lane == 0) S.off[n] = P.offsets[first + n];
+        if (lane == 0) { S.off[n] = P.offsets[first + n]; S.total_bytes = P.offsets[P.n_reads]; }
     }
     wp::sync();
 #ifndef C2B_EMU
@@ -1324,10 +1390,15 @@
     }
 #endif
     uint32_t fail = 0, route = 0;
+    diag_stage(P, S, 0, 0);
 #pragma unroll 1
     for (int x = 0; x < n; x++) {
         const int64_t off = S.off[x];
-        const int v = diag_read(P, S, first + x, off, (int)(S.off[x + 1] - off), S.ref[x], S.cnt[x], S.qw[x], A);
+        wp::wait_async();
+        wp::sync();
+        if (x + 1 < n) diag_stage(P, S, x + 1, (x + 1) & 1);
+        const int v = diag_read(P, S, first + x, S.raw[x & 1] + ((uintptr_t)(P.reads + off) & 15), (int)(S.off[x + 1] - off), S.ref[x],
+                                S.cnt[x], S.qw[x], A);
         if (v != DG_PROVED) fail |= 1u << x;
         if (v == DG_ROUTE) route |= 1u << x;
         wp::sync();
@@ -1361,7 +1432,8 @@
         wp::addg(&wb.diag_proved, proved); wp::addg(&wb.diag_listed, seen - proved);
         wp::addg(&wb.tier2, routed);
         wp::addg(&wb.routed, routed); wp::addg(&wb.kept, seen - proved - routed);
-    }
-}
-
-}
+        wp::addg(&wb.diag_popc, S.npop);
+    }
+}
+
+}
diff --git a/crispresso2_b200/engine.py b/crispresso2_b200/engine.py
--- a/crispresso2_b200/engine.py
+++ b/crispresso2_b200/engine.py
@@ -261,5 +261,10 @@
         self._check(self.L.c2b_route_counts(self.h, C.byref(a), C.byref(b)), "c2b_route_counts")
         return a.value, b.value
 
+    def diag_popcount_reads(self):
+        a = C.c_int64(0)
+        self._check(self.L.c2b_diag_popcount_reads(self.h, C.byref(a)), "c2b_diag_popcount_reads")
+        return a.value
+
     def launch_count(self):
         return int(self.L.c2b_launch_count(self.h))
diff --git a/include/c2b200.h b/include/c2b200.h
--- a/include/c2b200.h
+++ b/include/c2b200.h
@@ -174,6 +174,7 @@
 int  c2b_ring_counts(c2b_engine *e, int64_t *ring_pairs, int64_t *ring_fallbacks);
 int  c2b_diag_counts(c2b_engine *e, int64_t *proved, int64_t *tier1, int64_t *tier2);
 int  c2b_route_counts(c2b_engine *e, int64_t *routed, int64_t *kept);
+int  c2b_diag_popcount_reads(c2b_engine *e, int64_t *reads);
 
 int  c2b_counts_layout(const c2b_engine *e, int32_t *n_refs, int32_t *n_vec, int32_t *stride, int32_t *n_scal);
 int  c2b_counts_hist_layout(const c2b_engine *e, int32_t *n_hist, int32_t *hstride, int32_t *hist_zero);
```

After: 88.83 million (median of 6 runs). +7.2%, better.
